# JiehongLin/SAM-6D

Hardware: NVIDIA H100
Metric: poses/sec (higher is better)
Workload: dtype bf16

## Files before the change

### include/sam6d_b200.h

```cpp
#ifndef SAM6D_B200_H
#define SAM6D_B200_H

#ifdef __cplusplus
extern "C" {
#endif


int sam6d_fps(const float* xyz, int b, int n, int m, float* temp, int* idx, void* stream);
int sam6d_fps_single_cta(const float* xyz, int b, int n, int m, float* temp, int* idx, void* stream);

int sam6d_gather_points(const float* points, const int* idx, int b, int c, int n, int m, float* out, void* stream);

int sam6d_gather_rows(const float* src, const int* idx, int b, int n, int m, int c, long long src_bstride, float* out,
                      void* stream);
int sam6d_gather_rows_bf16_f32(const void* src, const int* idx, int b, int n, int m, int c, long long src_bstride, float* out,
                               void* stream);

int sam6d_ball_query(const float* new_xyz, const float* xyz, int b, int n, int m, float radius, int nsample, int* idx,
                     int* cnt, void* stream);
int sam6d_ball_query_pair(const float* new_xyz, const float* xyz, int b, int n, int m, float radius_a, int nsample_a,
                          float radius_b, int nsample_b, int* idx_a, int* idx_b, int* cnt_a, int* cnt_b, void* stream);

int sam6d_group_points(const float* points, const int* idx, int b, int c, int n, int np, int ns, float* out, void* stream);


int sam6d_gemm_f32(const float* A, const float* W, const float* bias, const float* R, float* C, int M, int N, int K,
                   long long lda, long long ldw, long long ldc, long long ldr, int batch, long long sA, long long sW,
                   long long sC, long long sR, float alpha, int relu, void* stream);

int sam6d_gemm_bf16(const void* A, int a_dtype, const void* W, int w_dtype, const float* bias, const float* R, void* C,
                    int c_dtype, int M, int N, int K, long long lda, long long ldw, long long ldc, long long ldr, int batch,
                    long long sA, long long sW, long long sC, long long sR, float alpha, int relu, void* stream);

int sam6d_gemm_tma(const void* A, const void* W, const float* bias, const void* R, void* C, int c_dtype, int M, int N, int K,
                   long long lda, long long ldw, long long ldc, long long ldr, float alpha, int act, void* stream);
int sam6d_gemm_tma_batched(const void* A, const void* W, const float* bias, const void* R, void* C, int c_dtype, int M, int N, int K,
                           long long lda, long long ldw, long long ldc, long long ldr, int batch, long long a_rpb, long long w_rpb,
                           long long c_bs, long long r_bs, float alpha, int act, void* stream);
int sam6d_gemm_tma_vt(const void* A, const void* W, const float* bias, void* C, int M, int N, int K, long long lda, long long ldw,
                      long long ldc, void* Vt, int vt_col0, int vt_S, int vt_N1, void* stream);
int sam6d_gemm_tma_vt2(const void* A, const void* W, const float* bias, void* C, int M, int N, int K, long long lda, long long ldw,
                       long long ldc, void* Vt, int vt_col0, int vt_col1, int vt_S, int vt_N1, void* C2, long long ldc2,
                       void* stream);


int sam6d_layernorm(const float* x, long long x_rpb, long long x_bstride, long long x_ld, float* y, long long y_rpb,
                    long long y_bstride, long long y_ld, const float* gamma, const float* beta, long long rows, int C,
                    float eps, void* stream);
int sam6d_layernorm_bf16(const float* x, long long x_rpb, long long x_bstride, long long x_ld, void* y, long long y_rpb,
                         long long y_bstride, long long y_ld, const float* gamma, const float* beta, long long rows, int C,
                         float eps, void* stream);
int sam6d_layernorm_bf16io(const void* x, long long x_rpb, long long x_bstride, long long x_ld, void* y, long long y_rpb,
                           long long y_bstride, long long y_ld, const float* gamma, const float* beta, long long rows, int C,
                           float eps, void* stream);
int sam6d_l2norm_rows(const float* x, long long x_rpb, long long x_bstride, long long x_ld, float* y, long long y_rpb,
                      long long y_bstride, long long y_ld, long long rows, int C, void* stream);
int sam6d_l2norm_rows_bf16(const float* x, long long x_rpb, long long x_bstride, long long x_ld, void* y, long long y_rpb,
                           long long y_bstride, long long y_ld, long long rows, int C, void* stream);
int sam6d_focus_rows(const float* x, long long x_rpb, long long x_bstride, long long x_ld, float* y, long long y_rpb,
                     long long y_bstride, long long y_ld, const float* softplus_scale, long long rows, int C, void* stream);
int sam6d_rigid_warp(const float* p, const float* R, const float* t, int b, int n, float* out, void* stream);
int sam6d_cloud_radius(const float* po, int b, int n, float* radius, void* stream);
int sam6d_scale_by_radius(const float* src, const float* radius, int b, long long per_batch, float* dst, void* stream);


int sam6d_geo_indices(const float* pts, int b, int S, float sigma_d, float factor_a, float* T, void* stream);
int sam6d_geo_embed_f32(const float* T, long long npairs, const float* div_term, const float* WaT, const float* WdT,
                        const float* bias, float* E, void* stream);

int sam6d_geo_embed_tc(const float* T, long long npairs, const float* div_term, const void* Wa_bf16, const void* Wd_bf16,
                       const float* bias, void* E, int e_is_bf16, void* stream);
int sam6d_geo_embed_dist_tc(const float* T, long long npairs, const float* div_term, const void* Wd_bf16, const float* bias, void* E,
                            void* stream);
int sam6d_geo_embed_lut(const float* T, long long clouds, int S, const void* tabA, int na, float inv_ha, const void* tabD, int nd,
                        float inv_hd, const void* far, const float* div_term, const void* WdT_bf16, const float* bias, void* E,
                        void* stream);


int sam6d_inputs_stage_a(const int* rle_cum, const int* rle_off, int P, int H, int W, const float* depth, double fx, double fy,
                         double cx, double cy, double thr, unsigned char* mask, int* stats, int cap, int* choose1, int* choose2,
                         float* cloud2, void* stream);
int sam6d_inputs_stage_b(const int* stats, const int* keep, int Q, int H, int W, int cap, const int* choose2, const float* cloud2,
                         const int* choose_idx, int ns, int S, const unsigned char* image, const unsigned char* mask, int mask_flag,
                         float* pts, long long* rgb_choose, float* rgb, unsigned char* rgb_u8, void* stream);

int sam6d_crop_resize_normalize(const unsigned char* images, const unsigned char* masks, const int* bbox, int Q, int H, int W, int S,
                                int mask_flag, float* rgb, unsigned char* rgb_u8, void* stream);


int sam6d_crop_resize_pad(const unsigned char* image, const float* masks, const int* boxes, int P, int H, int W, int T, float* rgb,
                          float* pmask, void* stream);
int sam6d_masked_patch_normalize(const float* tokens, long long tok_ld, long long tok_bs, const float* pmask, int P, int G, int patch,
                                 int C, float thresh, float* out_f32, void* out_bf16, unsigned char* valid, void* stream);
int sam6d_appearance_reduce(const float* sim, long long sim_ld, long long sim_bs, int P, int N, const unsigned char* qvalid, float thred,
                            float* appe, float* vis, void* stream);


int sam6d_query_translation(const float* masks, const int* depth, int N, int H, int W, const double* K, double depth_scale,
                            float* translate, void* stream);
int sam6d_project_template_iou(const float* poses, int T, const float* pointcloud, int O, int npc, const long long* best_pose,
                               const long long* pred_obj, const float* translate, const double* K, int N, int H, int W,
                               const long long* boxes, int* image_vu, int* xyxy, float* iou, unsigned char* ok, void* stream);


int sam6d_mask_rle_count(const float* masks, int n, int H, int W, int* col_cnt, int* band_off, int* rle_off, void* stream);
int sam6d_mask_rle_write(const float* masks, int n, int H, int W, const int* col_cnt, const int* band_off, const int* rle_off,
                         int* rle_cum, void* stream);


int sam6d_sam_pe_encode(const float* coords, const float* G, int rows, float* out, void* stream);
int sam6d_sam_mask_embed(const float* masks, const float* params, int B, float* out, void* stream);
int sam6d_sam_self_attn(const float* q, const float* k, const float* v, int B, int T, float* out, void* stream);
int sam6d_sam_tok2img_attn(const float* Q, const void* K, const void* V, long long kv_bs, int B, int T, int L, float* out, void* stream);
int sam6d_sam_img2tok_attn(const void* Q, long long q_bs, const float* Kt, const float* Vt, int B, int T, int L, void* out, void* stream);
int sam6d_sam_ln2d_gelu(const void* x, const float* gamma, const float* beta, long long rows, void* y, void* stream);
int sam6d_sam_mask_dot(const void* up, const float* hyper, int B, int G, float* masks, void* stream);
int sam6d_sam_mask_dot_range(const void* up, const float* hyper, int B, int G, int m0, int nm, float* masks, void* stream);
int sam6d_sam_mask_stats(const float* low, int N, int S, int big, int in_h, int in_w, int H, int W, float thr, float off, int* stats,
                         void* stream);
int sam6d_sam_mask_binarize(const float* low, const int* sel, int K, int S, int big, int in_h, int in_w, int H, int W, float thr,
                            unsigned char* out, void* stream);
int sam6d_sam_mask_upscale(const float* low, int N, int S, int big, int in_h, int in_w, int H, int W, float* out, void* stream);
int sam6d_sam_nms(const float* boxes, int N, float thr, unsigned char* keep, void* stream);


int sam6d_transformer_tail_bf16(const void* hid, long long ld_hid, const void* x, long long ld_x, const void* Wo, const float* bo,
                                const float* g1, const float* b1, const void* We, const float* be, const void* Ws, const float* bs,
                                const float* g2, const float* b2, void* out, long long ld_out, int M, float eps, void* stream);


int sam6d_rpe_scores(const void* E, int e_is_bf16, const float* U, long long u_ld, int B, int S, float* SP, void* stream);
int sam6d_rpe_scores_tc_ld(const void* E, const void* U, int B, int S, float* SP, int sp_ld, void* stream);
int sam6d_mha(const float* Q, long long q_ld, long long q_bs, const float* K, long long k_ld, long long k_bs, const float* V,
              long long v_ld, long long v_bs, const float* bias, int B, int H, int Sq, int Sk, float scale, float* O,
              long long o_ld, long long o_bs, void* stream);
int sam6d_attn_tc(const void* Q, long long q_ld, int q_col0, const void* K, long long k_ld, int k_col0, const void* Vt,
                  long long vt_ld, int B, int H, int Sq, int Sk, int head_dim, int bias_mode, const float* bias,
                  const void* rel_h, const float* rel_w, int Hs, int Ws, const float* bv, float scale, void* out,
                  int out_is_bf16, long long out_ld, void* stream);
int sam6d_attn_tc_bias_ld(const void* Q, long long q_ld, int q_col0, const void* K, long long k_ld, int k_col0, const void* Vt,
                          long long vt_ld, int B, int H, int Sq, int Sk, int head_dim, const float* bias, long long bias_ld,
                          float scale, void* out, int out_is_bf16, long long out_ld, void* stream);
int sam6d_attn_tc_ex(const void* Q, long long q_ld, int q_col0, const void* K, long long k_ld, int k_col0, const void* Vt,
                     long long vt_ld, int B, int H, int Sq, int Sk, int head_dim, float scale, int k_brows, int k_row0, int v_col0,
                     float* lse, void* out, int out_is_bf16, long long out_ld, void* stream);
int sam6d_attn_merge_key(const void* Q, long long q_ld, int q_col0, const void* K, long long k_ld, int k_col0, int k_brows,
                         int key_row, const void* Vt, long long vt_ld, int key_col, const float* lse, int B, int H, int Sq,
                         float scale, void* out, long long out_ld, void* stream);
int sam6d_transpose_tokens_bf16(const void* src, long long ld, int col0, int C, int nB, int L, int N1, void* out, void* stream);
int sam6d_linattn_kv(const float* Kf, long long k_ld, long long k_bs, const float* V, long long v_ld, long long v_bs, int B,
                     int H, int J, float* KV, float* KS, void* stream);
int sam6d_linattn_apply(const float* Qf, long long q_rpb, long long q_bs, long long q_ld, const float* KV, const float* KS,
                        int B, int H, float* X, long long x_bs, long long x_ld, void* stream);
int sam6d_linattn_kv_pack(const float* Kf, long long k_ld, long long k_bs, const float* V, long long v_ld, long long v_bs, int B,
                          int J, void* blob, float* KS, void* stream);
int sam6d_linattn_tc(const void* Q, long long q_ld, long long q_bs, const void* blob, const float* KS,
                     const float* softplus_scale, int B, int rpb, void* X, long long x_ld, long long x_bs, void* stream);

int sam6d_coarse_assign(const float* A, int B, int S, float* W, float* w1, void* stream);
int sam6d_coarse_sample(const float* W, int B, int L, const float* rand, int nr, int* idx, void* stream);
int sam6d_coarse_hypotheses(const int* idx, const float* pts1, const float* pts2, int B, int n, int n1, float* Rt,
                            float* resid, void* stream);
int sam6d_topk_smallest(const float* v, int B, int n, int k, int* out, void* stream);
int sam6d_coarse_select(const float* Rt, const int* top, int B, int n1, int n2, const float* pts1, const float* w1, int n,
                        const float* model, int nm, float* scores, float* R, float* t, void* stream);


int sam6d_pe_mlp_max(const float* pts, const int* idx, const int* cnt, int B, int N, int ns, const float* W1,
                     const float* B1, const float* W2, const float* B2, const float* W3, const float* B3, float* out,
                     int out_ld, int out_off, void* stream);
int sam6d_pe_mlp_max_tc(const float* pts, const int* idx, int B, int N, int ns, const float* W1, const float* B1,
                        const void* W2_bf16, const float* B2, const void* W3_bf16, const float* B3, void* out, int out_is_bf16,
                        int out_ld, int out_off, void* stream);
int sam6d_fine_assign(const float* A, int B, int S, int ld, float shift, const float* pts2, float* rsum, float* csum, float* cpart,
                      int* cpi, int* lab1, int* lab2, float* wts, float* pred, void* stream);
int sam6d_fine_pass_tc(const void* Fa, const void* Fb, int B, int S, float alpha, float shift, int mode, const float* row_f,
                       const float* col_f, int ld_f, const float* q4, float* out_inv, int* lab, float* wts, float* pred, void* stream);
int sam6d_fine_masked_points(const int* lab2, const float* pts2, int B, int S, int ld, float* q4, void* stream);
int sam6d_weighted_procrustes(const float* src, const float* ref, const float* wts, int B, int N, float weight_thresh,
                              float eps, float* R, float* t, void* stream);
int sam6d_pose_score(const float* pts1, const int* lab1, int B, int N, const float* R, const float* t, const float* model,
                     int nm, float dis_thres, const float* radius, float* score, float* t_scaled, void* stream);

int sam6d_bilinear_gather(const void* up, int up_is_bf16, const long long* choose, int B, int K, int G, int sub, int C, int H, int W,
                          float* out, void* stream);

int sam6d_attn_relpos(const float* qkv, long long tok_ld, int nW, int Hs, int Ws, int nH, int head_dim, const float* rel_h,
                      const float* rel_w, float scale, void* out, int out_is_bf16, long long out_ld, void* stream);

int sam6d_attn_global_tc(const void* qkv, long long ld, const void* Vt, long long vt_ld, const void* rel_blob, int B, int H, int grid,
                         float scale, void* out, int out_is_bf16, long long out_ld, void* stream);
int sam6d_attn_global_tc_ex(const void* qkv, long long ld, const void* Vt, long long vt_ld, const void* rel_blob, int B, int H, int grid,
                            int head_dim, float scale, void* out, int out_is_bf16, long long out_ld, void* stream);

int sam6d_template_score(const float* Qn, const float* Rn, int P, int O, int T, int C, float* sim_out, float* obj_score,
                         int* best_obj, float* best_score, int* best_tmpl, void* stream);


int sam6d_render_meshes(const float* verts, const int* faces, const int* mesh_info, int O, int n_verts, int n_faces,
                        const unsigned char* vcol, const float* uv, const unsigned char* tex, const long long* tex_off,
                        const float* base_color, const float* poses, int T, float fx, float fy, float cx, float cy, int H, int W,
                        float znear, float ambient, int* vrec, unsigned long long* vis, int* big, int big_cap, int* counters,
                        unsigned char* rgb, unsigned char* mask, void* xyz, int* tri, float* depth, void* stream);


int sam6d_conv2d_tc(const void* x, long long ldx, int B, int Hi, int Wi, int Cin, const void* w, int k, int stride, int Cout,
                    const float* bias, int silu, const void* r, long long ldr, long long r_bs, void* y, int y_is_f32, long long ldy,
                    long long y_bs, int Wy, int sy, int sx, int oy, int ox, void* stream);
int sam6d_yolo_stem(const unsigned char* img, int B, int H, int W, const float* w, const float* bias, void* out, void* stream);
int sam6d_yolo_sppf(void* buf, long long ld, int B, int H, int W, int C, void* stream);
int sam6d_yolo_upsample2x(const void* x, long long ldx, int B, int H, int W, int C, void* y, long long ldy, void* stream);
int sam6d_yolo_decode(const float* head, long long ld, long long bs, int B, int h0, int w0, int h1, int w1, int h2, int w2, float conf_thr,
                      float* cand, int* count, void* stream);
int sam6d_yolo_masks(const float* proto, int mh, int mw, const float* rows, long long row_ld, int N, int ih, int iw, float kx, float ky,
                     float* low, unsigned char* out, void* stream);

const char* sam6d_version(void);

#ifdef __cplusplus
}
#endif
#endif
```

### sam6d_b200/_lib.py

```python
import ctypes
import os
import re

_HERE = os.path.dirname(os.path.abspath(__file__))
HEADER = os.path.join(os.path.dirname(_HERE), "include", "sam6d_b200.h")
LIB_PATH = os.path.join(_HERE, "libsam6d_b200.so")

_CTYPES = {
    "int": ctypes.c_int,
    "long long": ctypes.c_longlong,
    "float": ctypes.c_float,
    "double": ctypes.c_double,
}


def parse_header(path: str = HEADER):
    text = open(path).read()
    text = re.sub(r"/\*.*?\*/", "", text, flags=re.S)
    protos = {}
    for m in re.finditer(r"(const char\*|int)\s+(sam6d_\w+)\s*\(([^)]*)\)\s*;", text):
        ret, name, args = m.group(1), m.group(2), m.group(3)
        argl = []
        for a in [x.strip() for x in args.split(",")]:
            if a in ("void", ""):
                continue
            if "*" in a:
                argl.append((ctypes.c_void_p, a.split("*")[-1].strip()))
            else:
                typ, nm = a.rsplit(" ", 1)
                argl.append((_CTYPES[typ.strip()], nm))
        protos[name] = (ctypes.c_char_p if ret != "int" else ctypes.c_int, argl)
    return protos


class Sam6dError(RuntimeError):
    pass


_lib = None
_protos = None


def lib():
    global _lib, _protos
    if _lib is None:
        if not os.path.exists(LIB_PATH):
            raise Sam6dError(
                f"{LIB_PATH} not found: build it with `python -m sam6d_b200.build` "
                "(or __graft_entry__.build()); sam6d_b200 has no CPU or eager fallback")
        _lib = ctypes.CDLL(LIB_PATH)
        _protos = parse_header()
        for name, (ret, args) in _protos.items():
            fn = getattr(_lib, name)
            fn.restype = ret
            fn.argtypes = [t for t, _ in args]
    return _lib


_launches = 0
_MULTI = {"sam6d_fine_assign": 6, "sam6d_coarse_select": 2, "sam6d_geo_embed_tc": 2, "sam6d_render_meshes": 4, "sam6d_yolo_masks": 2,
          "sam6d_mask_rle_count": 2}
_timed = {}


def launch_count() -> int:
    return _launches


def add_launches(n: int):
    global _launches
    _launches += int(n)


def time_kernel(name: str, enable: bool = True):
    if enable:
        _timed[name] = []
    else:
        _timed.pop(name, None)


def timed_events(name: str):
    return _timed.get(name, [])


def call(name: str, *args):
    global _launches
    fn = getattr(lib(), name)
    rec = _timed.get(name)
    if rec is not None:
        import torch
        e0, e1 = torch.cuda.Event(enable_timing=True), torch.cuda.Event(enable_timing=True)
        e0.record()
        rc = fn(*args)
        e1.record()
        rec.append((e0, e1))
    else:
        rc = fn(*args)
    _launches += _MULTI.get(name, 1)
    if rc != 0:
        if rc == -22:
            raise Sam6dError(f"{name}: invalid argument (see include/sam6d_b200.h)")
        raise Sam6dError(f"{name}: CUDA error {rc}")
    return rc


def version() -> str:
    return lib().sam6d_version().decode()
```

### sam6d_b200/csrc/fine_tc.cu

```cuda
#include <cuda.h>

#include "common.cuh"
#include "tc.cuh"

namespace {

constexpr int BM = 128, BN = 256, BK = 64, KB = 4, STAGES = 4;
constexpr int A_KB = BM * BK * 2, B_KB = BN * BK * 2;
constexpr int CONSUMERS = 256, NUM_THREADS = CONSUMERS + 128;
constexpr int SMEM_BYTES = KB * A_KB + STAGES * B_KB + 1024;
constexpr float LOG2E = 1.4426950408889634f;

struct FArgs {
  int B, S, mode, ld_f;
  float a2, s2;
  const float* row_f;
  const float* col_f;
  const float4* q4;
  float* out_inv;
  int* lab;
  float* wts; float* pred;
};

__device__ __forceinline__ float ex2(float x) {
  float y;
  asm("ex2.approx.ftz.f32 %0, %1;" : "=f"(y) : "f"(x));
  return y;
}

template <int MODE>
__global__ void __launch_bounds__(NUM_THREADS, 1) fine_pass_kernel(const __grid_constant__ CUtensorMap tmA, const __grid_constant__ CUtensorMap tmB, FArgs g) {
  extern __shared__ __align__(1024) uint8_t smem_raw[];
  uint8_t* smem = reinterpret_cast<uint8_t*>((reinterpret_cast<uintptr_t>(smem_raw) + 1023) & ~(uintptr_t)1023);
  uint8_t* a_res = smem;
  uint8_t* ring = smem + KB * A_KB;
  __shared__ __align__(8) uint64_t a_full, a_empty, full_bar[STAGES], empty_bar[STAGES];
  __shared__ float sc[2][BN];
  __shared__ __align__(16) float4 sq[2][BN];

  const int tid = threadIdx.x, warp = tid >> 5, lane = tid & 31;
  const int m_tiles = (g.S + BM - 1) / BM, n_tiles = (g.S + BN - 1) / BN;
  const int items = g.B * m_tiles;

  if (tid == 0) {
    tc::mbar_init(&a_full, 1); tc::mbar_init(&a_empty, CONSUMERS / 32);
    for (int s = 0; s < STAGES; ++s) { tc::mbar_init(&full_bar[s], 1); tc::mbar_init(&empty_bar[s], CONSUMERS / 32); }
    tc::mbar_fence_init();
    tc::tma_prefetch_desc(&tmA);
    tc::tma_prefetch_desc(&tmB);
  }
  __syncthreads();

  if (warp >= CONSUMERS / 32) {
    tc::producer_regs();
    if (tid == CONSUMERS) {
      long long gk = 0;
      int it = 0;
      for (int item = blockIdx.x; item < items; item += gridDim.x, ++it) {
        const int b = item / m_tiles, mt = item - b * m_tiles;
        tc::mbar_wait(&a_empty, (uint32_t)((it & 1) ^ 1));
        tc::mbar_arrive_expect_tx(&a_full, KB * A_KB);
        for (int kb = 0; kb < KB; ++kb) tc::tma_load_2d(&tmA, &a_full, a_res + kb * A_KB, kb * BK, b * g.S + mt * BM);
        for (int nt = 0; nt < n_tiles; ++nt)
          for (int kb = 0; kb < KB; ++kb, ++gk) {
            const int s = (int)(gk % STAGES);
            tc::mbar_wait(&empty_bar[s], (uint32_t)(((gk / STAGES) & 1) ^ 1));
            tc::mbar_arrive_expect_tx(&full_bar[s], B_KB);
            tc::tma_load_2d(&tmB, &full_bar[s], ring + s * B_KB, kb * BK, b * g.S + nt * BN);
          }
      }
    }
    return;
  }
  tc::consumer_regs();
  const int wg = warp >> 2, w = warp & 3;
  const uint32_t a_addr = tc::smem_u32(a_res) + wg * (64 * 128);
  long long gk = 0, tcount = 0;
  int it = 0;
  for (int item = blockIdx.x; item < items; item += gridDim.x, ++it) {
    const int b = item / m_tiles, mt = item - b * m_tiles;
    float rf[2] = {0.f, 0.f};
#pragma unroll
    for (int hr = 0; hr < 2; ++hr) {
      const int i = mt * BM + wg * 64 + tc::frag_row(2 * hr, w, lane);
      if (MODE != 0 && i < g.S) rf[hr] = g.row_f[(size_t)b * g.ld_f + i];
    }
    const float* cf = (MODE != 0) ? g.col_f + (size_t)b * g.ld_f : nullptr;
    const float4* q4 = (MODE == 2) ? g.q4 + (size_t)b * g.ld_f : nullptr;
    float sum[2] = {0.f, 0.f}, bv[2] = {-INFINITY, -INFINITY}, ws[2] = {0.f, 0.f}, px[2] = {0.f, 0.f}, py[2] = {0.f, 0.f}, pz[2] = {0.f, 0.f};
    int bi[2] = {0x7fffffff, 0x7fffffff};
    tc::mbar_wait(&a_full, (uint32_t)(it & 1));
    for (int nt = 0; nt < n_tiles; ++nt, ++tcount) {
      const int buf = (int)(tcount & 1);
      if (MODE != 0) {
        const int j = nt * BN + tid;
        sc[buf][tid] = (j < g.S) ? cf[j] : 0.f;
        if (MODE == 2) sq[buf][tid] = (j < g.S) ? q4[j] : make_float4(0.f, 0.f, 0.f, 0.f);
        tc::named_bar(1, CONSUMERS);
      }
      float acc[BN / 2];
      int prev = -1;
      for (int kb = 0; kb < KB; ++kb, ++gk) {
        const int s = (int)(gk % STAGES);
        tc::mbar_wait(&full_bar[s], (uint32_t)((gk / STAGES) & 1));
        const uint32_t b_addr = tc::smem_u32(ring + s * B_KB);
        tc::wg_fence();
#pragma unroll
        for (int k = 0; k < BK / 16; ++k)
          tc::wgmma_bf16<BN>(acc, tc::wg_desc(a_addr + kb * A_KB + k * 32), tc::wg_desc(b_addr + k * 32), (kb | k) ? 1u : 0u);
        tc::wg_commit();
        if (prev >= 0) {
          tc::wg_wait<1>();
          if (lane == 0) tc::mbar_arrive(&empty_bar[prev]);
        }
        prev = s;
      }
      tc::wg_wait<0>();
      if (lane == 0) tc::mbar_arrive(&empty_bar[prev]);
      if (nt == n_tiles - 1 && lane == 0) tc::mbar_arrive(&a_empty);
#pragma unroll
      for (int e = 0; e < BN / 2; ++e) {
        const int hr = (e >> 1) & 1, cl = tc::frag_col(e, lane), j = nt * BN + cl;
        const float ev = (j < g.S) ? ex2(fmaf(acc[e], g.a2, -g.s2)) : 0.f;
        if (MODE == 0) {
          sum[hr] += ev;
        } else {
          const float p = (ev * rf[hr]) * (ev * sc[buf][cl]);
          if (p > bv[hr]) { bv[hr] = p; bi[hr] = j; }
          if (MODE == 2) {
            const float4 q = sq[buf][cl];
            const float pm = p * q.w;
            ws[hr] += pm; px[hr] = fmaf(pm, q.x, px[hr]); py[hr] = fmaf(pm, q.y, py[hr]); pz[hr] = fmaf(pm, q.z, pz[hr]);
          }
        }
      }
    }
#pragma unroll
    for (int hr = 0; hr < 2; ++hr) {
      const int i = mt * BM + wg * 64 + tc::frag_row(2 * hr, w, lane);
      if (MODE == 0) {
        const float t = tc::quad_sum(sum[hr]);
        if ((lane & 3) == 0 && i < g.S) g.out_inv[(size_t)b * g.ld_f + i] = 1.f / t;
      } else {
#pragma unroll
        for (int o = 1; o <= 2; o <<= 1) {
          const float ov = __shfl_xor_sync(0xffffffffu, bv[hr], o);
          const int oi = __shfl_xor_sync(0xffffffffu, bi[hr], o);
          if (ov > bv[hr] || (ov == bv[hr] && oi < bi[hr])) { bv[hr] = ov; bi[hr] = oi; }
        }
        float ww = 0.f, qx = 0.f, qy = 0.f, qz = 0.f;
        if (MODE == 2) { ww = tc::quad_sum(ws[hr]); qx = tc::quad_sum(px[hr]); qy = tc::quad_sum(py[hr]); qz = tc::quad_sum(pz[hr]); }
        if ((lane & 3) == 0 && i < g.S) {
          int lb = bi[hr];
          if (lb == 0x7fffffff) lb = 0;
          g.lab[(size_t)b * g.S + i] = lb;
          if (MODE == 2 && i >= 1) {
            if (lb == 0) { ww = 0.f; qx = 0.f; qy = 0.f; qz = 0.f; }
            const size_t o = (size_t)b * (g.S - 1) + (i - 1);
            const float d = ww + 1e-6f;
            g.wts[o] = ww;
            g.pred[o * 3 + 0] = qx / d; g.pred[o * 3 + 1] = qy / d; g.pred[o * 3 + 2] = qz / d;
          }
        }
      }
    }
  }
}

typedef CUresult (*EncodeFn)(CUtensorMap*, CUtensorMapDataType, cuuint32_t, void*, const cuuint64_t*, const cuuint64_t*,
                             const cuuint32_t*, const cuuint32_t*, CUtensorMapInterleave, CUtensorMapSwizzle,
                             CUtensorMapL2promotion, CUtensorMapFloatOOBfill);
EncodeFn f_get_encode() {
  static EncodeFn fn = nullptr;
  if (!fn) {
    void* p = nullptr;
    cudaDriverEntryPointQueryResult q;
    if (cudaGetDriverEntryPoint("cuTensorMapEncodeTiled", &p, cudaEnableDefault, &q) != cudaSuccess || q != cudaDriverEntryPointSuccess)
      return nullptr;
    fn = reinterpret_cast<EncodeFn>(p);
  }
  return fn;
}
int f_make_map(CUtensorMap* map, const void* ptr, long long rows, int box_rows) {
  EncodeFn enc = f_get_encode();
  if (!enc) return 999;
  cuuint64_t gdim[2] = {256, (cuuint64_t)rows};
  cuuint64_t gstride[1] = {512};
  cuuint32_t box[2] = {64, (cuuint32_t)box_rows};
  cuuint32_t estr[2] = {1, 1};
  CUresult r = enc(map, CU_TENSOR_MAP_DATA_TYPE_BFLOAT16, 2, const_cast<void*>(ptr), gdim, gstride, box, estr,
                   CU_TENSOR_MAP_INTERLEAVE_NONE, CU_TENSOR_MAP_SWIZZLE_128B, CU_TENSOR_MAP_L2_PROMOTION_L2_256B,
                   CU_TENSOR_MAP_FLOAT_OOB_FILL_NONE);
  return r == CUDA_SUCCESS ? 0 : 1000 + (int)r;
}

__global__ void fine_masked_points_kernel(const int* __restrict__ lab2, const float* __restrict__ pts2, int S, int ld, float4* __restrict__ q4) {
  const int b = blockIdx.y, j = blockIdx.x * blockDim.x + threadIdx.x;
  if (j >= ld) return;
  float4 q = make_float4(0.f, 0.f, 0.f, 0.f);
  if (j >= 1 && j < S && lab2[(size_t)b * S + j] > 0) {
    const float* p = pts2 + ((size_t)b * (S - 1) + (j - 1)) * 3;
    q = make_float4(p[0], p[1], p[2], 1.f);
  }
  q4[(size_t)b * ld + j] = q;
}

}

S6_API int sam6d_fine_pass_tc(const void* Fa, const void* Fb, int B, int S, float alpha, float shift, int mode, const float* row_f,
                              const float* col_f, int ld_f, const float* q4, float* out_inv, int* lab, float* wts, float* pred,
                              void* stream) {
  S6_REQUIRE(Fa && Fb && B >= 0 && S >= 2 && mode >= 0 && mode <= 2 && ld_f >= S);
  S6_REQUIRE(((reinterpret_cast<uintptr_t>(Fa) | reinterpret_cast<uintptr_t>(Fb)) & 15) == 0 && (long long)B * S < 2000000000LL);
  if (mode == 0) S6_REQUIRE(out_inv != nullptr);
  if (mode >= 1) S6_REQUIRE(row_f && col_f && lab);
  if (mode == 2) S6_REQUIRE(q4 && wts && pred && (reinterpret_cast<uintptr_t>(q4) & 15) == 0);
  if (B == 0) return 0;
  CUtensorMap tmA, tmB;
  int rc = f_make_map(&tmA, Fa, (long long)B * S, BM);
  if (rc) return rc;
  rc = f_make_map(&tmB, Fb, (long long)B * S, BN);
  if (rc) return rc;
  int dev = 0, sms = 0;
  S6_CHECK(cudaGetDevice(&dev));
  S6_CHECK(cudaDeviceGetAttribute(&sms, cudaDevAttrMultiProcessorCount, dev));
  const int items = B * s6_cdiv(S, BM);
  const int grid = items < sms ? items : sms;
  FArgs g{B, S, mode, ld_f, alpha * LOG2E, shift * LOG2E, row_f, col_f, reinterpret_cast<const float4*>(q4), out_inv, lab, wts, pred};
  cudaStream_t st = s6_stream(stream);
#define FINE_LAUNCH(M)                                                                                              \
  do {                                                                                                              \
    S6_CHECK(cudaFuncSetAttribute(fine_pass_kernel<M>, cudaFuncAttributeMaxDynamicSharedMemorySize, SMEM_BYTES));   \
    fine_pass_kernel<M><<<grid, NUM_THREADS, SMEM_BYTES, st>>>(tmA, tmB, g);                                        \
  } while (0)
  if (mode == 0) FINE_LAUNCH(0); else if (mode == 1) FINE_LAUNCH(1); else FINE_LAUNCH(2);
#undef FINE_LAUNCH
  S6_LAUNCH_CHECK();
  return 0;
}

S6_API int sam6d_fine_masked_points(const int* lab2, const float* pts2, int B, int S, int ld, float* q4, void* stream) {
  S6_REQUIRE(lab2 && pts2 && q4 && B >= 0 && S >= 2 && ld >= S && (reinterpret_cast<uintptr_t>(q4) & 15) == 0);
  if (B == 0) return 0;
  dim3 grid(s6_cdiv(ld, 256), B);
  fine_masked_points_kernel<<<grid, 256, 0, s6_stream(stream)>>>(lab2, pts2, S, ld, reinterpret_cast<float4*>(q4));
  S6_LAUNCH_CHECK();
  return 0;
}
```

### sam6d_b200/csrc/pe_tc.cu

```cuda
#include "tc.cuh"

namespace {

constexpr int ROWS = 128;
constexpr int SLAB = ROWS * 128;
constexpr int W2_SLAB = 64 * 128;
constexpr int W3_SLAB = 128 * 128;
constexpr int SMEM_BYTES = 2 * SLAB + W3_SLAB + 1024;
constexpr int NUM_THREADS = 128;

__device__ __forceinline__ void worker_bar() { asm volatile("bar.sync 1, 128;" ::: "memory"); }

__device__ __forceinline__ void st_feat(float* p, float v) { *p = v; }
__device__ __forceinline__ void st_feat(__nv_bfloat16* p, float v) { *p = __float2bfloat16(v); }

template <int NS, typename OT>
__global__ void __launch_bounds__(NUM_THREADS, 4) pe_tc_kernel(const float* __restrict__ pts, const int* __restrict__ idx, int N,
                                                               long long total_points,
                                                               const float* __restrict__ W1, const float* __restrict__ B1,
                                                               const __nv_bfloat16* __restrict__ W2, const float* __restrict__ B2,
                                                               const __nv_bfloat16* __restrict__ W3, const float* __restrict__ B3,
                                                               OT* __restrict__ out, int out_ld, int out_off) {
  extern __shared__ __align__(1024) uint8_t smem_raw[];
  uint8_t* smem = reinterpret_cast<uint8_t*>((reinterpret_cast<uintptr_t>(smem_raw) + 1023) & ~(uintptr_t)1023);
  uint8_t* a1 = smem;
  uint8_t* a2 = a1 + SLAB;
  uint8_t* w3s = a2 + SLAB;
  __shared__ __align__(16) float w1s[32 * 8];
  __shared__ __align__(16) float b1s[32], b2s[64], b3s[128];

  const int tid = threadIdx.x, warp = tid >> 5, lane = tid & 31;
  constexpr int PPT = ROWS / NS;
  const long long ntiles = (total_points + PPT - 1) / PPT;

  for (int e = tid; e < 32 * 8; e += NUM_THREADS) { int r = e >> 3, c = e & 7; w1s[e] = (c < 6) ? W1[r * 6 + c] : 0.f; }
  if (tid < 32) b1s[tid] = B1[tid];
  if (tid < 64) b2s[tid] = B2[tid];
  if (tid < 128) b3s[tid] = B3[tid];
  for (int u = tid; u < 64 * 4; u += NUM_THREADS) {
    const int n = u >> 2, c = (u & 3) << 3;
    *reinterpret_cast<uint4*>(a1 + tc::sw128_offset(n, 32 + c)) = *reinterpret_cast<const uint4*>(W2 + n * 32 + c);
  }
  for (int u = tid; u < 128 * 8; u += NUM_THREADS) {
    const int n = u >> 3, c = (u & 7) << 3;
    *reinterpret_cast<uint4*>(w3s + tc::sw128_offset(n, c)) = *reinterpret_cast<const uint4*>(W3 + n * 64 + c);
  }
  tc::fence_proxy_async_smem();
  __syncthreads();

  {
    const int r = tid;
    const uint32_t a1_addr = tc::smem_u32(a1), a2_addr = tc::smem_u32(a2), w2_addr = tc::smem_u32(a1) + 64, w3_addr = tc::smem_u32(w3s);
    auto load_idx = [&](long long tile) -> int {
      const long long gp = tile * PPT + r / NS;
      return (tile < ntiles && gp < total_points) ? __ldg(idx + gp * NS + (r % NS)) : -1;
    };
    auto load_x = [&](long long tile, int j, float (&xx)[6]) {
      const long long gp = tile * PPT + r / NS;
      if (j >= 0) {
        const long long b = gp / N;
        const float* pi = pts + gp * 3;
        const float* pj = pts + (b * N + j) * 3;
        const float jx = __ldg(pj), jy = __ldg(pj + 1), jz = __ldg(pj + 2);
        xx[0] = jx - __ldg(pi); xx[1] = jy - __ldg(pi + 1); xx[2] = jz - __ldg(pi + 2); xx[3] = jx; xx[4] = jy; xx[5] = jz;
      } else {
#pragma unroll
        for (int e = 0; e < 6; ++e) xx[e] = 0.f;
      }
    };
    float xn[6];
    load_x(blockIdx.x, load_idx(blockIdx.x), xn);
    int jn = load_idx((long long)blockIdx.x + gridDim.x);
    for (long long tile = blockIdx.x; tile < ntiles; tile += gridDim.x) {
      {
        float x[6];
#pragma unroll
        for (int e = 0; e < 6; ++e) x[e] = xn[e];
        uint8_t* row_ptr = a1 + r * 128;
#pragma unroll
        for (int c = 0; c < 4; ++c) {
          uint32_t w[4];
#pragma unroll
          for (int q = 0; q < 4; ++q) {
            float h[2];
#pragma unroll
            for (int e = 0; e < 2; ++e) {
              const int o = c * 8 + q * 2 + e;
              const float4 wa = *reinterpret_cast<const float4*>(&w1s[o * 8]);
              const float2 wb = *reinterpret_cast<const float2*>(&w1s[o * 8 + 4]);
              float a = b1s[o];
              a = fmaf(wa.x, x[0], a); a = fmaf(wa.y, x[1], a); a = fmaf(wa.z, x[2], a);
              a = fmaf(wa.w, x[3], a); a = fmaf(wb.x, x[4], a); a = fmaf(wb.y, x[5], a);
              h[e] = fmaxf(a, 0.f);
            }
            w[q] = tc::pack_bf16(h[0], h[1]);
          }
          *reinterpret_cast<uint4*>(row_ptr + ((c ^ (r & 7)) << 4)) = make_uint4(w[0], w[1], w[2], w[3]);
        }
        tc::fence_proxy_async_smem();
        worker_bar();
      }
#pragma unroll
      for (int blk = 0; blk < 2; ++blk) {
        float acc[32];
        tc::wg_fence();
#pragma unroll
        for (int k = 0; k < 2; ++k)
          tc::wgmma_bf16<64>(acc, tc::wg_desc(a1_addr + blk * (64 * 128) + k * 32), tc::wg_desc(w2_addr + k * 32), k ? 1u : 0u);
        tc::wg_commit();
        tc::wg_wait<0>();
#pragma unroll
        for (int i = 0; i < 32; i += 2) {
          const int row = blk * 64 + tc::frag_row(i, warp, lane), col = tc::frag_col(i, lane);
          *reinterpret_cast<uint32_t*>(a2 + tc::sw128_offset(row, col)) =
              tc::pack_bf16(fmaxf(acc[i] + b2s[col], 0.f), fmaxf(acc[i + 1] + b2s[col + 1], 0.f));
        }
      }
      tc::fence_proxy_async_smem();
      worker_bar();
      load_x(tile + gridDim.x, jn, xn);
      jn = load_idx(tile + 2LL * gridDim.x);
#pragma unroll
      for (int blk = 0; blk < 2; ++blk) {
        float acc[64];
        tc::wg_fence();
#pragma unroll
        for (int k = 0; k < 4; ++k)
          tc::wgmma_bf16<128>(acc, tc::wg_desc(w3_addr + blk * (64 * 128) + k * 32), tc::wg_desc(a2_addr + k * 32), k ? 1u : 0u);
        tc::wg_commit();
        tc::wg_wait<0>();
#pragma unroll
        for (int hr = 0; hr < 2; ++hr) {
          const int ch = blk * 64 + tc::frag_row(2 * hr, warp, lane);
          const float bias = b3s[ch];
#pragma unroll
          for (int p = 0; p < PPT; ++p) {
            constexpr int JG = NS / 8;
            float m = -INFINITY;
#pragma unroll
            for (int j = p * JG; j < (p + 1) * JG; ++j) m = fmaxf(m, fmaxf(acc[4 * j + 2 * hr], acc[4 * j + 2 * hr + 1]));
            m = tc::quad_max(m);
            const long long p_out = tile * PPT + p;
            if ((lane & 3) == 0 && p_out < total_points) st_feat(out + p_out * out_ld + out_off + ch, fmaxf(m + bias, 0.f));
          }
        }
      }
    }
  }
}

}

S6_API int sam6d_pe_mlp_max_tc(const float* pts, const int* idx, int B, int N, int ns, const float* W1, const float* B1,
                               const void* W2_bf16, const float* B2, const void* W3_bf16, const float* B3, void* out, int out_is_bf16,
                               int out_ld, int out_off, void* stream) {
  S6_REQUIRE(pts && idx && W1 && B1 && W2_bf16 && B2 && W3_bf16 && B3 && out && B >= 0 && N > 0);
  S6_REQUIRE(ns == 32 || ns == 64);
  if (B == 0) return 0;
  int dev = 0, sms = 0;
  S6_CHECK(cudaGetDevice(&dev));
  S6_CHECK(cudaDeviceGetAttribute(&sms, cudaDevAttrMultiProcessorCount, dev));
  const long long total = (long long)B * N;
  const long long ntiles = (total + (128 / ns) - 1) / (128 / ns);
  cudaStream_t st = s6_stream(stream);
  const __nv_bfloat16* W2 = reinterpret_cast<const __nv_bfloat16*>(W2_bf16);
  const __nv_bfloat16* W3 = reinterpret_cast<const __nv_bfloat16*>(W3_bf16);
#define PE_LAUNCH(NSV, OT)                                                                                                          \
  do {                                                                                                                              \
    S6_CHECK(cudaFuncSetAttribute(pe_tc_kernel<NSV, OT>, cudaFuncAttributeMaxDynamicSharedMemorySize, SMEM_BYTES));                 \
                       \
    S6_CHECK(cudaFuncSetAttribute(pe_tc_kernel<NSV, OT>, cudaFuncAttributePreferredSharedMemoryCarveout, 100));                     \
       \
       \
    const int per_sm = 4;                                                                                                           \
    const int grid = (int)(ntiles < (long long)sms * per_sm ? ntiles : (long long)sms * per_sm);                                    \
    pe_tc_kernel<NSV, OT><<<grid, NUM_THREADS, SMEM_BYTES, st>>>(pts, idx, N, total, W1, B1, W2, B2, W3, B3,                         \
                                                                 reinterpret_cast<OT*>(out), out_ld, out_off);                      \
  } while (0)
  if (ns == 32) { if (out_is_bf16) PE_LAUNCH(32, __nv_bfloat16); else PE_LAUNCH(32, float); }
  else { if (out_is_bf16) PE_LAUNCH(64, __nv_bfloat16); else PE_LAUNCH(64, float); }
#undef PE_LAUNCH
  S6_LAUNCH_CHECK();
  return 0;
}
```

### sam6d_b200/ops.py

```python
import ctypes
from typing import Optional, Tuple

import torch

from . import _lib

Tensor = torch.Tensor


def _check(t: Tensor, dtype, name: str, ndim: Optional[int] = None):
    if not isinstance(t, torch.Tensor):
        raise RuntimeError(f"{name} must be a torch.Tensor")
    if not t.is_cuda:
        raise RuntimeError(f"{name} must be a CUDA tensor (CPU not supported)")
    if t.dtype != dtype:
        raise RuntimeError(f"{name} must be {dtype}, got {t.dtype}")
    if not t.is_contiguous():
        raise RuntimeError(f"{name} must be contiguous")
    if ndim is not None and t.dim() != ndim:
        raise RuntimeError(f"{name} must have {ndim} dims, got {t.dim()}")


def _p(t: Optional[Tensor]):
    return ctypes.c_void_p(0 if t is None else t.data_ptr())


def _s():
    return ctypes.c_void_p(torch.cuda.current_stream().cuda_stream)


def _ll(v):
    return ctypes.c_longlong(int(v))


def _f(v):
    return ctypes.c_float(float(v))


def furthest_point_sampling(xyz: Tensor, m: int) -> Tensor:
    _check(xyz, torch.float32, "points", 3)
    b, n, c = xyz.shape
    if c != 3:
        raise RuntimeError("points must be (B,N,3)")
    idx = torch.zeros(b, m, dtype=torch.int32, device=xyz.device)
    temp = torch.empty(b, n, dtype=torch.float32, device=xyz.device) if n > 4096 else None
    _lib.call("sam6d_fps", _p(xyz), b, n, int(m), _p(temp), _p(idx), _s())
    return idx


def furthest_point_sampling_single_cta(xyz: Tensor, m: int) -> Tensor:
    _check(xyz, torch.float32, "points", 3)
    b, n, _ = xyz.shape
    idx = torch.zeros(b, m, dtype=torch.int32, device=xyz.device)
    temp = torch.empty(b, n, dtype=torch.float32, device=xyz.device)
    _lib.call("sam6d_fps_single_cta", _p(xyz), b, n, int(m), _p(temp), _p(idx), _s())
    return idx


def gather_points(points: Tensor, idx: Tensor) -> Tensor:
    _check(points, torch.float32, "points", 3)
    _check(idx, torch.int32, "idx", 2)
    b, c, n = points.shape
    m = idx.shape[1]
    out = torch.zeros(b, c, m, dtype=torch.float32, device=points.device)
    _lib.call("sam6d_gather_points", _p(points), _p(idx), b, c, n, m, _p(out), _s())
    return out


def gather_rows(src: Tensor, idx: Tensor, n_rows: Optional[int] = None) -> Tensor:
    _check(src, torch.float32, "src", 3)
    _check(idx, torch.int32, "idx", 2)
    b, n, c = src.shape
    m = idx.shape[1]
    out = torch.empty(b, m, c, dtype=torch.float32, device=src.device)
    _lib.call("sam6d_gather_rows", _p(src), _p(idx), b, n, m, c, _ll(n * c), _p(out), _s())
    return out


def ball_query(new_xyz: Tensor, xyz: Tensor, radius: float, nsample: int, return_count: bool = False):
    _check(new_xyz, torch.float32, "new_xyz", 3)
    _check(xyz, torch.float32, "xyz", 3)
    b, m, _ = new_xyz.shape
    n = xyz.shape[1]
    idx = torch.zeros(b, m, nsample, dtype=torch.int32, device=xyz.device)
    cnt = torch.zeros(b, m, dtype=torch.int32, device=xyz.device) if return_count else None
    _lib.call("sam6d_ball_query", _p(new_xyz), _p(xyz), b, n, m, _f(radius), int(nsample), _p(idx), _p(cnt), _s())
    return (idx, cnt) if return_count else idx


def ball_query_pair(new_xyz: Tensor, xyz: Tensor, ra: float, nsa: int, rb: float, nsb: int):
    _check(new_xyz, torch.float32, "new_xyz", 3)
    _check(xyz, torch.float32, "xyz", 3)
    b, m, _ = new_xyz.shape
    n = xyz.shape[1]
    dev = xyz.device
    ia = torch.empty(b, m, nsa, dtype=torch.int32, device=dev)
    ib = torch.empty(b, m, nsb, dtype=torch.int32, device=dev)
    ca = torch.empty(b, m, dtype=torch.int32, device=dev)
    cb = torch.empty(b, m, dtype=torch.int32, device=dev)
    _lib.call("sam6d_ball_query_pair", _p(new_xyz), _p(xyz), b, n, m, _f(ra), int(nsa), _f(rb), int(nsb), _p(ia), _p(ib), _p(ca),
              _p(cb), _s())
    return ia, ca, ib, cb


def group_points(points: Tensor, idx: Tensor) -> Tensor:
    _check(points, torch.float32, "points", 3)
    _check(idx, torch.int32, "idx", 3)
    b, c, n = points.shape
    _, npnt, ns = idx.shape
    out = torch.zeros(b, c, npnt, ns, dtype=torch.float32, device=points.device)
    _lib.call("sam6d_group_points", _p(points), _p(idx), b, c, n, npnt, ns, _p(out), _s())
    return out


def gemm(A: Tensor, W: Tensor, bias: Optional[Tensor] = None, residual: Optional[Tensor] = None,
         out: Optional[Tensor] = None, relu=False, alpha: float = 1.0) -> Tensor:
    _check(A, torch.float32, "A", 2)
    _check(W, torch.float32, "W", 2)
    M, K = A.shape
    N = W.shape[0]
    if W.shape[1] != K:
        raise RuntimeError("gemm: inner dimensions differ")
    if out is None:
        out = torch.empty(M, N, dtype=torch.float32, device=A.device)
    _lib.call("sam6d_gemm_f32", _p(A), _p(W), _p(bias), _p(residual), _p(out), M, N, K, _ll(K), _ll(K), _ll(N), _ll(N),
              1, _ll(0), _ll(0), _ll(0), _ll(0), _f(alpha), int(relu), _s())
    return out


def gemm_raw(A_ptr, W_ptr, bias, R_ptr, C_ptr, M, N, K, lda, ldw, ldc, ldr, batch=1, sA=0, sW=0, sC=0, sR=0,
             alpha=1.0, relu=False):
    _lib.call("sam6d_gemm_f32", ctypes.c_void_p(A_ptr), ctypes.c_void_p(W_ptr), _p(bias), ctypes.c_void_p(R_ptr or 0),
              ctypes.c_void_p(C_ptr), int(M), int(N), int(K), _ll(lda), _ll(ldw), _ll(ldc), _ll(ldr), int(batch), _ll(sA),
              _ll(sW), _ll(sC), _ll(sR), _f(alpha), int(relu), _s())


_DT = {torch.float32: 0, torch.bfloat16: 1}


def gemm_tc_raw(A_ptr, a_dt, W_ptr, w_dt, bias, R_ptr, C_ptr, c_dt, M, N, K, lda, ldw, ldc, ldr, batch=1, sA=0, sW=0, sC=0, sR=0,
                alpha=1.0, relu=False):
    _lib.call("sam6d_gemm_bf16", ctypes.c_void_p(A_ptr), int(a_dt), ctypes.c_void_p(W_ptr), int(w_dt), _p(bias),
              ctypes.c_void_p(R_ptr or 0), ctypes.c_void_p(C_ptr), int(c_dt), int(M), int(N), int(K), _ll(lda), _ll(ldw), _ll(ldc),
              _ll(ldr), int(batch), _ll(sA), _ll(sW), _ll(sC), _ll(sR), _f(alpha), int(relu), _s())


def gemm_tc(A: Tensor, W: Tensor, bias: Optional[Tensor] = None, residual: Optional[Tensor] = None, out: Optional[Tensor] = None,
            relu: bool = False, alpha: float = 1.0, out_dtype=torch.float32) -> Tensor:
    for t, n in ((A, "A"), (W, "W")):
        if t.dtype not in _DT:
            raise RuntimeError(f"{n} must be float32 or bfloat16")
        _check(t, t.dtype, n, 2)
    M, K = A.shape
    N = W.shape[0]
    if W.shape[1] != K:
        raise RuntimeError("gemm: inner dimensions differ")
    if out is None:
        out = torch.empty(M, N, dtype=out_dtype, device=A.device)
    gemm_tc_raw(A.data_ptr(), _DT[A.dtype], W.data_ptr(), _DT[W.dtype], bias, residual.data_ptr() if residual is not None else 0,
                out.data_ptr(), _DT[out.dtype], M, N, K, K, K, N, N, alpha=alpha, relu=relu)
    return out


def gemm_tma(A: Tensor, W: Tensor, bias: Optional[Tensor] = None, residual: Optional[Tensor] = None, out: Optional[Tensor] = None,
             act: int = 0, alpha: float = 1.0, out_dtype=torch.float32) -> Tensor:
    _check(A, torch.bfloat16, "A", 2)
    _check(W, torch.bfloat16, "W", 2)
    M, K = A.shape
    N = W.shape[0]
    if W.shape[1] != K:
        raise RuntimeError("gemm: inner dimensions differ")
    Nout = N // 2 if act == ACT_SWIGLU else N
    if out is None:
        out = torch.empty(M, Nout, dtype=torch.bfloat16 if act == ACT_SWIGLU else out_dtype, device=A.device)
    if residual is not None:
        _check(residual, out.dtype, "residual", 2)
    _lib.call("sam6d_gemm_tma", _p(A), _p(W), _p(bias), _p(residual), _p(out), _DT[out.dtype], M, N, K, _ll(K), _ll(K), _ll(Nout), _ll(N),
              _f(alpha), int(act), _s())
    return out


ACT_SWIGLU = 3


def pack_swiglu_rows(t: Tensor, block: int = 128) -> Tensor:
    H = t.shape[0] // 2
    if t.shape[0] != 2 * H or H % block:
        raise ValueError(f"SwiGLU w12 needs 2H rows with H % {block} == 0, got {t.shape[0]}")
    rest = t.shape[1:]
    return t.reshape(2, H // block, block, *rest).transpose(0, 1).reshape(2 * H, *rest).contiguous()


_VT_CACHE = {}


def _vt_buffer(rows: int, n1: int, device, slot: int) -> Tensor:
    key = (rows, n1, str(device), slot, torch.cuda.current_stream(device).cuda_stream)
    buf = _VT_CACHE.get(key)
    if buf is None:
        if len(_VT_CACHE) > 64:
            _VT_CACHE.clear()
        buf = torch.zeros(rows, n1, dtype=torch.bfloat16, device=device)
        _VT_CACHE[key] = buf
    return buf


def gemm_tma_vt(A: Tensor, W: Tensor, bias: Tensor, vt_col0: int, S: int, slot: int = 0) -> Tuple[Tensor, Tensor]:
    _check(A, torch.bfloat16, "A", 2)
    _check(W, torch.bfloat16, "W", 2)
    M, K = A.shape
    N = W.shape[0]
    if W.shape[1] != K or M % S or not (0 < vt_col0 < N):
        raise RuntimeError("gemm_tma_vt: shape mismatch")
    n1 = (S + 15) // 16 * 16
    out = torch.empty(M, vt_col0, dtype=torch.bfloat16, device=A.device)
    vt = _vt_buffer((M // S) * (N - vt_col0), n1, A.device, slot)
    _lib.call("sam6d_gemm_tma_vt", _p(A), _p(W), _p(bias), _p(out), M, N, K, _ll(K), _ll(K), _ll(vt_col0), _p(vt), int(vt_col0), int(S),
              int(n1), _s())
    return out, vt


def gemm_tma_vt2(A: Tensor, W: Tensor, bias: Tensor, vt_col0: int, vt_col1: int, S: int, slot: int = 0) -> Tuple[Tensor, Tensor, Tensor]:
    _check(A, torch.bfloat16, "A", 2)
    _check(W, torch.bfloat16, "W", 2)
    M, K = A.shape
    N = W.shape[0]
    if W.shape[1] != K or M % S or not (0 < vt_col0 < vt_col1 < N):
        raise RuntimeError("gemm_tma_vt2: shape mismatch")
    n1 = (S + 15) // 16 * 16
    out = torch.empty(M, vt_col0, dtype=torch.bfloat16, device=A.device)
    out2 = torch.empty(M, N - vt_col1, dtype=torch.bfloat16, device=A.device)
    vt = _vt_buffer((M // S) * (vt_col1 - vt_col0), n1, A.device, slot)
    _lib.call("sam6d_gemm_tma_vt2", _p(A), _p(W), _p(bias), _p(out), M, N, K, _ll(K), _ll(K), _ll(vt_col0), _p(vt), int(vt_col0),
              int(vt_col1), int(S), int(n1), _p(out2), _ll(N - vt_col1), _s())
    return out, vt, out2


def layernorm_raw(x_ptr, x_view, y_ptr, y_view, gamma: Tensor, beta: Tensor, rows: int, C: int, eps: float = 1e-5):
    _lib.call("sam6d_layernorm", ctypes.c_void_p(x_ptr), _ll(x_view[0]), _ll(x_view[1]), _ll(x_view[2]),
              ctypes.c_void_p(y_ptr), _ll(y_view[0]), _ll(y_view[1]), _ll(y_view[2]), _p(gamma), _p(beta), _ll(rows), int(C),
              _f(eps), _s())


def layernorm(x: Tensor, gamma: Tensor, beta: Tensor, eps: float = 1e-5, out: Optional[Tensor] = None) -> Tensor:
    _check(x, torch.float32, "x")
    C = x.shape[-1]
    rows = x.numel() // C
    if out is None:
        out = torch.empty_like(x)
    layernorm_raw(x.data_ptr(), (rows, 0, C), out.data_ptr(), (rows, 0, C), gamma, beta, rows, C, eps)
    return out


def layernorm_bf16(x: Tensor, gamma: Tensor, beta: Tensor, eps: float = 1e-5) -> Tensor:
    _check(x, torch.float32, "x")
    C = x.shape[-1]
    rows = x.numel() // C
    out = torch.empty(x.shape, dtype=torch.bfloat16, device=x.device)
    _lib.call("sam6d_layernorm_bf16", _p(x), _ll(rows), _ll(0), _ll(C), _p(out), _ll(rows), _ll(0), _ll(C), _p(gamma), _p(beta),
              _ll(rows), int(C), _f(eps), _s())
    return out


def layernorm_bf16io(x: Tensor, gamma: Tensor, beta: Tensor, eps: float = 1e-5, out: Optional[Tensor] = None) -> Tensor:
    _check(x, torch.bfloat16, "x")
    C = x.shape[-1]
    rows = x.numel() // C
    if out is None:
        out = torch.empty_like(x)
    _lib.call("sam6d_layernorm_bf16io", _p(x), _ll(max(rows, 1)), _ll(0), _ll(C), _p(out), _ll(max(rows, 1)), _ll(0), _ll(C),
              _p(gamma), _p(beta), _ll(rows), int(C), _f(eps), _s())
    return out


def transformer_tail_bf16(hid: Tensor, x: Tensor, wo: Tensor, bo: Tensor, g1: Tensor, b1: Tensor, we: Tensor, be: Tensor, ws: Tensor,
                          bs: Tensor, g2: Tensor, b2: Tensor, out: Optional[Tensor] = None, eps: float = 1e-5) -> Tensor:
    _check(hid, torch.bfloat16, "hid", 2)
    _check(x, torch.bfloat16, "x", 2)
    M = hid.shape[0]
    if hid.shape[1] != 256 or x.shape != hid.shape or wo.shape != (256, 256) or we.shape != (512, 256) or ws.shape != (256, 512):
        raise RuntimeError("transformer_tail_bf16: d_model 256, hidden 512")
    for w in (wo, we, ws):
        _check(w, torch.bfloat16, "weight", 2)
    if out is None:
        out = torch.empty_like(hid)
    _check(out, torch.bfloat16, "out", 2)
    _lib.call("sam6d_transformer_tail_bf16", _p(hid), _ll(256), _p(x), _ll(256), _p(wo), _p(bo), _p(g1), _p(b1), _p(we), _p(be), _p(ws),
              _p(bs), _p(g2), _p(b2), _p(out), _ll(256), int(M), _f(eps), _s())
    return out


def gather_rows_bf16_f32(src: Tensor, idx: Tensor) -> Tensor:
    _check(src, torch.bfloat16, "src", 3)
    _check(idx, torch.int32, "idx", 2)
    b, n, c = src.shape
    m = idx.shape[1]
    out = torch.empty(b, m, c, dtype=torch.float32, device=src.device)
    _lib.call("sam6d_gather_rows_bf16_f32", _p(src), _p(idx), b, n, m, c, _ll(n * c), _p(out), _s())
    return out


def gather_rows_bf16(src: Tensor, idx: Tensor) -> Tensor:
    _check(src, torch.bfloat16, "src", 3)
    _check(idx, torch.int32, "idx", 2)
    b, n, c = src.shape
    m = idx.shape[1]
    out = torch.empty(b, m, c, dtype=torch.bfloat16, device=src.device)
    _lib.call("sam6d_gather_rows", _p(src), _p(idx), b, n, m, c // 2, _ll(n * c // 2), _p(out), _s())
    return out


def l2norm_rows(x: Tensor) -> Tensor:
    _check(x, torch.float32, "x")
    C = x.shape[-1]
    rows = x.numel() // C
    out = torch.empty_like(x)
    _lib.call("sam6d_l2norm_rows", _p(x), _ll(rows), _ll(0), _ll(C), _p(out), _ll(rows), _ll(0), _ll(C), _ll(rows), C, _s())
    return out


def l2norm_rows_bf16(x: Tensor) -> Tensor:
    _check(x, torch.float32, "x")
    C = x.shape[-1]
    rows = x.numel() // C
    out = torch.empty(x.shape, dtype=torch.bfloat16, device=x.device)
    _lib.call("sam6d_l2norm_rows_bf16", _p(x), _ll(max(rows, 1)), _ll(0), _ll(C), _p(out), _ll(max(rows, 1)), _ll(0), _ll(C), _ll(rows), C,
              _s())
    return out


def gemm_tma_batched(A: Tensor, W: Tensor, out: Tensor, M: int, N: int, ldc: int, c_bs: int, alpha: float = 1.0,
                     bias: Optional[Tensor] = None, residual: Optional[Tensor] = None, ldr: int = 0, r_bs: int = 0) -> Tensor:
    _check(A, torch.bfloat16, "A", 3)
    _check(W, torch.bfloat16, "W")
    batch, a_rows, K = A.shape
    shared = W.dim() == 2
    if W.shape[-1] != K or a_rows < M or (not shared and (W.shape[0] != batch or W.shape[1] < N)) or (shared and W.shape[0] != N):
        raise RuntimeError("gemm_tma_batched: shape mismatch")
    if residual is not None and residual.dtype != out.dtype:
        raise RuntimeError("gemm_tma_batched: the residual must have the output's element type")
    _lib.call("sam6d_gemm_tma_batched", _p(A), _p(W), _p(bias), _p(residual), _p(out), _DT[out.dtype], int(M), int(N), int(K), _ll(K),
              _ll(K), _ll(ldc), _ll(ldr), int(batch), _ll(a_rows), _ll(0 if shared else W.shape[1]), _ll(c_bs), _ll(r_bs), _f(alpha), 0,
              _s())
    return out


def focus_rows_raw(x_ptr, x_view, y_ptr, y_view, sp_scale: Tensor, rows: int, C: int):
    _lib.call("sam6d_focus_rows", ctypes.c_void_p(x_ptr), _ll(x_view[0]), _ll(x_view[1]), _ll(x_view[2]),
              ctypes.c_void_p(y_ptr), _ll(y_view[0]), _ll(y_view[1]), _ll(y_view[2]), _p(sp_scale), _ll(rows), int(C), _s())


def rigid_warp(p: Tensor, R: Tensor, t: Tensor) -> Tensor:
    _check(p, torch.float32, "p", 3)
    _check(R, torch.float32, "R", 3)
    _check(t, torch.float32, "t", 2)
    out = torch.empty_like(p)
    _lib.call("sam6d_rigid_warp", _p(p), _p(R), _p(t), p.shape[0], p.shape[1], _p(out), _s())
    return out


def cloud_radius(po: Tensor) -> Tensor:
    _check(po, torch.float32, "dense_po", 3)
    r = torch.empty(po.shape[0], dtype=torch.float32, device=po.device)
    _lib.call("sam6d_cloud_radius", _p(po), po.shape[0], po.shape[1], _p(r), _s())
    return r


def scale_by_radius(x: Tensor, radius: Tensor) -> Tensor:
    _check(x, torch.float32, "x")
    _check(radius, torch.float32, "radius", 1)
    out = torch.empty_like(x)
    b = x.shape[0]
    _lib.call("sam6d_scale_by_radius", _p(x), _p(radius), b, _ll(x.numel() // max(b, 1)), _p(out), _s())
    return out


def geo_indices(pts: Tensor, sigma_d: float, factor_a: float) -> Tensor:
    _check(pts, torch.float32, "points", 3)
    b, s, _ = pts.shape
    T = torch.empty(b, s, s, 4, dtype=torch.float32, device=pts.device)
    _lib.call("sam6d_geo_indices", _p(pts), b, s, _f(sigma_d), _f(factor_a), _p(T), _s())
    return T


def geo_embed_f32(T: Tensor, div_term: Tensor, WaT: Tensor, WdT: Tensor, bias: Tensor) -> Tensor:
    _check(T, torch.float32, "T", 4)
    b, s, _, _ = T.shape
    E = torch.empty(b, s, s, 256, dtype=torch.float32, device=T.device)
    _lib.call("sam6d_geo_embed_f32", _p(T), _ll(b * s * s), _p(div_term), _p(WaT), _p(WdT), _p(bias), _p(E), _s())
    return E


def geo_embed_tc(T: Tensor, div_term: Tensor, Wa_bf16: Tensor, Wd_bf16: Tensor, bias: Tensor, out_dtype=torch.bfloat16) -> Tensor:
    _check(T, torch.float32, "T", 4)
    _check(Wa_bf16, torch.bfloat16, "Wa", 2)
    _check(Wd_bf16, torch.bfloat16, "Wd", 2)
    b, s, _, _ = T.shape
    E = torch.empty(b, s, s, 256, dtype=out_dtype, device=T.device)
    _lib.call("sam6d_geo_embed_tc", _p(T), _ll(b * s * s), _p(div_term), _p(Wa_bf16), _p(Wd_bf16), _p(bias), _p(E),
              int(out_dtype == torch.bfloat16), _s())
    return E


def geo_embed_dist_tc(T: Tensor, div_term: Tensor, Wd_bf16: Tensor, bias: Tensor) -> Tensor:
    if T.dtype != torch.float32 or not T.is_cuda or not T.is_contiguous() or T.shape[-1] != 4:
        raise RuntimeError("T must be a contiguous CUDA float32 tensor (..., 4)")
    _check(Wd_bf16, torch.bfloat16, "Wd", 2)
    n = T.numel() // 4
    E = torch.empty(*T.shape[:-1], 256, dtype=torch.bfloat16, device=T.device)
    _lib.call("sam6d_geo_embed_dist_tc", _p(T), _ll(n), _p(div_term), _p(Wd_bf16), _p(bias), _p(E), _s())
    return E


def geo_embed_lut(T: Tensor, tabA: Tensor, inv_ha: float, tabD: Tensor, inv_hd: float, far: Tensor, div_term: Tensor, WdT_bf16: Tensor,
                  bias: Tensor) -> Tensor:
    _check(T, torch.float32, "T", 4)
    _check(tabA, torch.bfloat16, "tabA", 2)
    _check(tabD, torch.bfloat16, "tabD", 2)
    _check(far, torch.bfloat16, "far", 4)
    _check(WdT_bf16, torch.bfloat16, "WdT", 2)
    b, s, _, _ = T.shape
    if far.shape != (b, 2, s, 256) or tabA.shape[1] != 256 or tabD.shape[1] != 256 or T.shape[3] != 4:
        raise RuntimeError("geo_embed_lut: shape mismatch")
    E = torch.empty(b, s, s, 256, dtype=torch.bfloat16, device=T.device)
    _lib.call("sam6d_geo_embed_lut", _p(T), _ll(b), s, _p(tabA), tabA.shape[0], _f(inv_ha), _p(tabD), tabD.shape[0], _f(inv_hd), _p(far),
              _p(div_term), _p(WdT_bf16), _p(bias), _p(E), _s())
    return E


def rpe_scores(E: Tensor, U: Tensor, u_ptr: Optional[int] = None, u_ld: int = 1024) -> Tensor:
    if E.dtype not in (torch.float32, torch.bfloat16):
        raise RuntimeError("E must be float32 or bfloat16")
    _check(E, E.dtype, "E", 4)
    if u_ptr is None:
        _check(U, torch.float32, "U", 4)
        u_ptr = U.data_ptr()
    B, S = E.shape[0], E.shape[1]
    SP = torch.empty(B, 4, S, S, dtype=torch.float32, device=E.device)
    _lib.call("sam6d_rpe_scores", _p(E), int(E.dtype == torch.bfloat16), ctypes.c_void_p(u_ptr), _ll(u_ld), B, S, _p(SP), _s())
    return SP


def rpe_scores_tc(E: Tensor, U: Tensor, ld: Optional[int] = None) -> Tensor:
    _check(E, torch.bfloat16, "E", 4)
    _check(U, torch.bfloat16, "U", 2)
    B, S = E.shape[0], E.shape[1]
    if U.shape != (B * S, 1024) or E.shape[3] != 256 or E.shape[2] != S:
        raise RuntimeError("rpe_scores_tc: E (B,S,S,256), U (B*S,1024)")
    ld = S if ld is None else ld
    SP = torch.empty(B, 4, S, ld, dtype=torch.float32, device=E.device)
    _lib.call("sam6d_rpe_scores_tc_ld", _p(E), _p(U), B, S, _p(SP), int(ld), _s())
    return SP


def rpe_scores_tc_padded(E: Tensor, U: Tensor) -> Tensor:
    return rpe_scores_tc(E, U, ld=(E.shape[1] + 15) // 16 * 16)


def attn_tc_padded_bias(Q: Tensor, q_col0: int, K: Tensor, k_col0: int, Vt: Tensor, B: int, H: int, Sq: int, Sk: int, D: int,
                        scale: float, bias: Tensor, out_dtype=torch.bfloat16) -> Tensor:
    _check(Q, torch.bfloat16, "Q", 2)
    _check(K, torch.bfloat16, "K", 2)
    _check(Vt, torch.bfloat16, "Vt", 2)
    _check(bias, torch.float32, "bias", 4)
    if bias.shape[:3] != (B, H, Sq) or bias.shape[3] < Sk or bias.shape[3] % 4:
        raise RuntimeError("attn_tc_padded_bias: bias (B,H,Sq,ld), ld >= Sk, ld % 4 == 0")
    out = torch.empty(B * Sq, H * D, dtype=out_dtype, device=Q.device)
    _lib.call("sam6d_attn_tc_bias_ld", _p(Q), _ll(Q.shape[1]), int(q_col0), _p(K), _ll(K.shape[1]), int(k_col0), _p(Vt), _ll(Vt.shape[1]),
              int(B), int(H), int(Sq), int(Sk), int(D), _p(bias), _ll(bias.shape[3]), _f(scale), _p(out),
              int(out_dtype == torch.bfloat16), _ll(H * D), _s())
    return out


def mha_raw(q_ptr, q_ld, q_bs, k_ptr, k_ld, k_bs, v_ptr, v_ld, v_bs, bias: Optional[Tensor], B, H, Sq, Sk, scale,
            o_ptr, o_ld, o_bs):
    _lib.call("sam6d_mha", ctypes.c_void_p(q_ptr), _ll(q_ld), _ll(q_bs), ctypes.c_void_p(k_ptr), _ll(k_ld), _ll(k_bs),
              ctypes.c_void_p(v_ptr), _ll(v_ld), _ll(v_bs), _p(bias), int(B), int(H), int(Sq), int(Sk), _f(scale),
              ctypes.c_void_p(o_ptr), _ll(o_ld), _ll(o_bs), _s())


def pack_rel_pos(rel_h: Tensor, rel_w: Tensor, slab_rows: int = 32) -> Tensor:
    D = rel_h.shape[1]
    DS = (D + 63) // 64
    if rel_h.shape[0] > slab_rows or rel_w.shape[0] > slab_rows:
        raise RuntimeError("pack_rel_pos: table has more rows than the slab")
    blob = torch.zeros(2 * DS * slab_rows * 64, dtype=torch.bfloat16, device=rel_h.device)
    j = torch.arange(slab_rows, device=rel_h.device).view(slab_rows, 1)
    c = torch.arange(D, device=rel_h.device).view(1, D)
    off = j * 64 + ((((c % 64) // 8) ^ (j % 8)) * 8) + (c % 8)
    for t, tab in enumerate((rel_h, rel_w)):
        n = tab.shape[0]
        idx = ((t * DS + c // 64) * slab_rows * 64 + off)[:n]
        blob[idx.reshape(-1)] = tab.to(torch.bfloat16).reshape(-1)
    return blob


def attn_global_tc(qkv: Tensor, vt: Tensor, rel_blob: Tensor, B: int, H: int, grid: int, scale: float, out_dtype=torch.bfloat16,
                   D: int = 80) -> Tensor:
    _check(qkv, torch.bfloat16, "qkv", 2)
    _check(vt, torch.bfloat16, "vt", 2)
    _check(rel_blob, torch.bfloat16, "rel_blob", 1)
    L = grid * grid
    out = torch.empty(B * L, H * D, dtype=out_dtype, device=qkv.device)
    _lib.call("sam6d_attn_global_tc_ex", _p(qkv), _ll(qkv.shape[1]), _p(vt), _ll(vt.shape[1]), _p(rel_blob), int(B), int(H), int(grid),
              int(D), _f(scale), _p(out), int(out_dtype == torch.bfloat16), _ll(H * D), _s())
    return out


def attn_tc(Q: Tensor, q_col0: int, K: Tensor, k_col0: int, Vt: Tensor, B: int, H: int, Sq: int, Sk: int, D: int, scale: float,
            bias: Optional[Tensor] = None, rel: Optional[tuple] = None, bv: Optional[Tensor] = None,
            out_dtype=torch.float32) -> Tensor:
    _check(Q, torch.bfloat16, "Q", 2)
    _check(K, torch.bfloat16, "K", 2)
    _check(Vt, torch.bfloat16, "Vt", 2)
    mode, rh, rw, Hs, Ws = 0, None, None, 0, 0
    if bias is not None:
        _check(bias, torch.float32, "bias", 4)
        mode = 1
    elif rel is not None:
        rh, Hs, Ws = rel
        mode = 2
    out = torch.empty(B * Sq, H * D, dtype=out_dtype, device=Q.device)
    _lib.call("sam6d_attn_tc", _p(Q), _ll(Q.shape[1]), int(q_col0), _p(K), _ll(K.shape[1]), int(k_col0), _p(Vt), _ll(Vt.shape[1]),
              int(B), int(H), int(Sq), int(Sk), int(D), mode, _p(bias), _p(rh), _p(rw), int(Hs), int(Ws), _p(bv), _f(scale), _p(out),
              int(out_dtype == torch.bfloat16), _ll(H * D), _s())
    return out


def attn_tc_ex(Q: Tensor, q_col0: int, K: Tensor, k_col0: int, Vt: Tensor, B: int, H: int, Sq: int, Sk: int, D: int, scale: float,
               k_brows: int, k_row0: int = 0, v_col0: int = 0, want_lse: bool = False, out_dtype=torch.bfloat16):
    _check(Q, torch.bfloat16, "Q", 2)
    _check(K, torch.bfloat16, "K", 2)
    _check(Vt, torch.bfloat16, "Vt", 2)
    out = torch.empty(B * Sq, H * D, dtype=out_dtype, device=Q.device)
    lse = torch.empty(B, H, Sq, dtype=torch.float32, device=Q.device) if want_lse else None
    _lib.call("sam6d_attn_tc_ex", _p(Q), _ll(Q.shape[1]), int(q_col0), _p(K), _ll(K.shape[1]), int(k_col0), _p(Vt), _ll(Vt.shape[1]),
              int(B), int(H), int(Sq), int(Sk), int(D), _f(scale), int(k_brows), int(k_row0), int(v_col0), _p(lse), _p(out),
              int(out_dtype == torch.bfloat16), _ll(H * D), _s())
    return out, lse


def attn_merge_key(Q: Tensor, q_col0: int, K: Tensor, k_col0: int, k_brows: int, key_row: int, Vt: Tensor, key_col: int, lse: Tensor,
                   B: int, H: int, Sq: int, scale: float, out: Tensor) -> Tensor:
    _check(out, torch.bfloat16, "out", 2)
    _check(lse, torch.float32, "lse", 3)
    _lib.call("sam6d_attn_merge_key", _p(Q), _ll(Q.shape[1]), int(q_col0), _p(K), _ll(K.shape[1]), int(k_col0), int(k_brows), int(key_row),
              _p(Vt), _ll(Vt.shape[1]), int(key_col), _p(lse), int(B), int(H), int(Sq), _f(scale), _p(out), _ll(out.shape[1]), _s())
    return out


def transpose_tokens(src: Tensor, col0: int, C: int, nB: int, L: int) -> Tensor:
    _check(src, torch.bfloat16, "src", 2)
    N1 = (L + 15) // 16 * 16
    out = torch.empty(nB * C, N1, dtype=torch.bfloat16, device=src.device)
    _lib.call("sam6d_transpose_tokens_bf16", _p(src), _ll(src.shape[1]), int(col0), int(C), int(nB), int(L), int(N1), _p(out), _s())
    return out


def linattn_kv_raw(k_ptr, k_ld, k_bs, v_ptr, v_ld, v_bs, B, H, J, KV: Tensor, KS: Tensor):
    _lib.call("sam6d_linattn_kv", ctypes.c_void_p(k_ptr), _ll(k_ld), _ll(k_bs), ctypes.c_void_p(v_ptr), _ll(v_ld), _ll(v_bs),
              int(B), int(H), int(J), _p(KV), _p(KS), _s())


def linattn_apply_raw(q_ptr, q_rpb, q_bs, q_ld, KV: Tensor, KS: Tensor, B, H, x_ptr, x_bs, x_ld):
    _lib.call("sam6d_linattn_apply", ctypes.c_void_p(q_ptr), _ll(q_rpb), _ll(q_bs), _ll(q_ld), _p(KV), _p(KS), int(B), int(H),
              ctypes.c_void_p(x_ptr), _ll(x_bs), _ll(x_ld), _s())


def linattn_kv_pack_raw(k_ptr, k_ld, k_bs, v_ptr, v_ld, v_bs, B, J, device):
    blob = torch.empty(B, 4 * 64 * 64, dtype=torch.bfloat16, device=device)
    KS = torch.empty(B, 4, 64, dtype=torch.float32, device=device)
    _lib.call("sam6d_linattn_kv_pack", ctypes.c_void_p(k_ptr), _ll(k_ld), _ll(k_bs), ctypes.c_void_p(v_ptr), _ll(v_ld), _ll(v_bs),
              int(B), int(J), _p(blob), _p(KS), _s())
    return blob, KS


def linattn_tc_raw(q_ptr, q_ld, q_bs, blob: Tensor, KS: Tensor, sp_scale: Tensor, B, rpb, x_ptr, x_ld, x_bs):
    _lib.call("sam6d_linattn_tc", ctypes.c_void_p(q_ptr), _ll(q_ld), _ll(q_bs), _p(blob), _p(KS), _p(sp_scale), int(B), int(rpb),
              ctypes.c_void_p(x_ptr), _ll(x_ld), _ll(x_bs), _s())


def coarse_assign(A: Tensor) -> Tuple[Tensor, Tensor]:
    _check(A, torch.float32, "atten", 3)
    B, S, _ = A.shape
    n = S - 1
    W = torch.empty(B, n * n, dtype=torch.float32, device=A.device)
    w1 = torch.empty(B, n, dtype=torch.float32, device=A.device)
    _lib.call("sam6d_coarse_assign", _p(A), B, S, _p(W), _p(w1), _s())
    return W, w1


def coarse_sample(W: Tensor, rand: Tensor) -> Tensor:
    _check(W, torch.float32, "W", 2)
    _check(rand, torch.float32, "rand", 2)
    B, L = W.shape
    nr = rand.shape[1]
    idx = torch.empty(B, nr, dtype=torch.int32, device=W.device)
    _lib.call("sam6d_coarse_sample", _p(W), B, L, _p(rand), nr, _p(idx), _s())
    return idx


def coarse_hypotheses(idx: Tensor, pts1: Tensor, pts2: Tensor) -> Tuple[Tensor, Tensor]:
    _check(idx, torch.int32, "idx", 2)
    _check(pts1, torch.float32, "pts1", 3)
    _check(pts2, torch.float32, "pts2", 3)
    B, n, _ = pts1.shape
    n1 = idx.shape[1] // 3
    Rt = torch.empty(B, n1, 12, dtype=torch.float32, device=idx.device)
    resid = torch.empty(B, n1, dtype=torch.float32, device=idx.device)
    _lib.call("sam6d_coarse_hypotheses", _p(idx), _p(pts1), _p(pts2), B, n, n1, _p(Rt), _p(resid), _s())
    return Rt, resid


def topk_smallest(v: Tensor, k: int) -> Tensor:
    _check(v, torch.float32, "v", 2)
    B, n = v.shape
    out = torch.empty(B, k, dtype=torch.int32, device=v.device)
    _lib.call("sam6d_topk_smallest", _p(v), B, n, int(k), _p(out), _s())
    return out


def coarse_select(Rt: Tensor, top: Tensor, pts1: Tensor, w1: Tensor, model: Tensor):
    _check(Rt, torch.float32, "Rt", 3)
    _check(top, torch.int32, "top", 2)
    _check(model, torch.float32, "model", 3)
    B, n1, _ = Rt.shape
    n2 = top.shape[1]
    n = pts1.shape[1]
    scores = torch.empty(B, n2, dtype=torch.float32, device=Rt.device)
    R = torch.empty(B, 3, 3, dtype=torch.float32, device=Rt.device)
    t = torch.empty(B, 3, dtype=torch.float32, device=Rt.device)
    _lib.call("sam6d_coarse_select", _p(Rt), _p(top), B, n1, n2, _p(pts1), _p(w1), n, _p(model), model.shape[1], _p(scores),
              _p(R), _p(t), _s())
    return R, t, scores


def pe_mlp_max(pts: Tensor, idx: Tensor, cnt: Tensor, weights, out: Tensor, out_off: int):
    _check(pts, torch.float32, "pts", 3)
    _check(idx, torch.int32, "idx", 3)
    _check(cnt, torch.int32, "cnt", 2)
    B, N, _ = pts.shape
    ns = idx.shape[2]
    W1, B1, W2, B2, W3, B3 = weights
    _lib.call("sam6d_pe_mlp_max", _p(pts), _p(idx), _p(cnt), B, N, ns, _p(W1), _p(B1), _p(W2), _p(B2), _p(W3), _p(B3),
              _p(out), out.shape[-1], int(out_off), _s())


def pe_mlp_max_tc(pts: Tensor, idx: Tensor, weights, out: Tensor, out_off: int):
    _check(pts, torch.float32, "pts", 3)
    _check(idx, torch.int32, "idx", 3)
    B, N, _ = pts.shape
    ns = idx.shape[2]
    W1, B1, W2, B2, W3, B3 = weights
    _check(W2, torch.bfloat16, "W2", 2)
    _check(W3, torch.bfloat16, "W3", 2)
    if out.dtype not in (torch.float32, torch.bfloat16):
        raise RuntimeError("pe_mlp_max_tc: out must be float32 or bfloat16")
    _lib.call("sam6d_pe_mlp_max_tc", _p(pts), _p(idx), B, N, ns, _p(W1), _p(B1), _p(W2), _p(B2), _p(W3), _p(B3), _p(out),
              int(out.dtype == torch.bfloat16), out.shape[-1], int(out_off), _s())


def fine_assign(A: Tensor, pts2: Tensor, shift: float):
    if A.dim() != 3 or A.dtype != torch.float32 or not A.is_cuda:
        raise RuntimeError("atten must be a CUDA fp32 (B,S,S) tensor")
    _check(pts2, torch.float32, "pts2", 3)
    B, S, _ = A.shape
    if A.stride(2) != 1 or A.stride(0) != S * A.stride(1) or A.stride(1) % 4 or A.data_ptr() % 16:
        ld = (S + 3) // 4 * 4
        store = torch.empty(B, S, ld, dtype=torch.float32, device=A.device)
        store[:, :, :S] = A
        A = store[:, :, :S]
    ld = A.stride(1)
    dev = A.device
    tiles = (S + 31) // 32
    if tiles < 4:
        raise RuntimeError("fine_assign: S >= 97 required")
    rsum = torch.empty(B, ld, dtype=torch.float32, device=dev)
    csum = torch.empty(B, ld, dtype=torch.float32, device=dev)
    cpart = torch.empty(B, tiles, ld, dtype=torch.float32, device=dev)
    cpi = torch.empty(B, tiles, ld, dtype=torch.int32, device=dev)
    lab1 = torch.zeros(B, S, dtype=torch.int32, device=dev)
    lab2 = torch.zeros(B, S, dtype=torch.int32, device=dev)
    wts = torch.empty(B, S - 1, dtype=torch.float32, device=dev)
    pred = torch.empty(B, S - 1, 3, dtype=torch.float32, device=dev)
    _lib.call("sam6d_fine_assign", _p(A), B, S, int(ld), _f(shift), _p(pts2), _p(rsum), _p(csum), _p(cpart), _p(cpi), _p(lab1),
              _p(lab2), _p(wts), _p(pred), _s())
    return lab1, lab2, wts, pred


def fine_assign_tc(f1n: Tensor, f2n: Tensor, pts2: Tensor, alpha: float):
    _check(f1n, torch.bfloat16, "f1n", 3)
    _check(f2n, torch.bfloat16, "f2n", 3)
    _check(pts2, torch.float32, "pts2", 3)
    B, S, C = f1n.shape
    if C != 256 or f2n.shape != f1n.shape or pts2.shape[1] != S - 1:
        raise RuntimeError("fine_assign_tc: (B,S,256) tokens and (B,S-1,3) points expected")
    dev = f1n.device
    ld = (S + 3) // 4 * 4
    rinv = torch.empty(B, ld, dtype=torch.float32, device=dev)
    cinv = torch.empty(B, ld, dtype=torch.float32, device=dev)
    q4 = torch.empty(B, ld, 4, dtype=torch.float32, device=dev)
    lab1 = torch.zeros(B, S, dtype=torch.int32, device=dev)
    lab2 = torch.zeros(B, S, dtype=torch.int32, device=dev)
    wts = torch.empty(B, S - 1, dtype=torch.float32, device=dev)
    pred = torch.empty(B, S - 1, 3, dtype=torch.float32, device=dev)
    a, sh = _f(alpha), _f(alpha)
    _lib.call("sam6d_fine_pass_tc", _p(f1n), _p(f2n), B, S, a, sh, 0, None, None, ld, None, _p(rinv), None, None, None, _s())
    _lib.call("sam6d_fine_pass_tc", _p(f2n), _p(f1n), B, S, a, sh, 0, None, None, ld, None, _p(cinv), None, None, None, _s())
    _lib.call("sam6d_fine_pass_tc", _p(f2n), _p(f1n), B, S, a, sh, 1, _p(cinv), _p(rinv), ld, None, None, _p(lab2), None, None, _s())
    _lib.call("sam6d_fine_masked_points", _p(lab2), _p(pts2), B, S, ld, _p(q4), _s())
    _lib.call("sam6d_fine_pass_tc", _p(f1n), _p(f2n), B, S, a, sh, 2, _p(rinv), _p(cinv), ld, _p(q4), None, _p(lab1), _p(wts), _p(pred),
              _s())
    return lab1, lab2, wts, pred


def weighted_procrustes(src: Tensor, ref: Tensor, wts: Tensor, weight_thresh: float = 0.0, eps: float = 1e-5):
    _check(src, torch.float32, "src", 3)
    _check(ref, torch.float32, "ref", 3)
    _check(wts, torch.float32, "weights", 2)
    B, N, _ = src.shape
    R = torch.empty(B, 3, 3, dtype=torch.float32, device=src.device)
    t = torch.empty(B, 3, dtype=torch.float32, device=src.device)
    _lib.call("sam6d_weighted_procrustes", _p(src), _p(ref), _p(wts), B, N, _f(weight_thresh), _f(eps), _p(R), _p(t), _s())
    return R, t


def pose_score(pts1: Tensor, lab1: Tensor, R: Tensor, t: Tensor, model: Tensor, radius: Tensor, dis_thres: float = 0.15):
    _check(pts1, torch.float32, "pts1", 3)
    _check(lab1, torch.int32, "lab1", 2)
    B, N, _ = pts1.shape
    score = torch.empty(B, dtype=torch.float32, device=pts1.device)
    ts = torch.empty(B, 3, dtype=torch.float32, device=pts1.device)
    _lib.call("sam6d_pose_score", _p(pts1), _p(lab1), B, N, _p(R), _p(t), _p(model), model.shape[1], _f(dis_thres),
              _p(radius), _p(score), _p(ts), _s())
    return score, ts


def attn_relpos(qkv: Tensor, nW: int, Hs: int, Ws: int, nH: int, rel_h: Tensor, rel_w: Tensor, scale: float,
                out_dtype=torch.float32) -> Tensor:
    _check(qkv, torch.float32, "qkv", 2)
    _check(rel_h, torch.float32, "rel_pos_h", 2)
    _check(rel_w, torch.float32, "rel_pos_w", 2)
    T, C3 = qkv.shape
    C = C3 // 3
    if T != nW * Hs * Ws or rel_h.shape[0] != 2 * Hs - 1 or rel_w.shape[0] != 2 * Ws - 1:
        raise RuntimeError("attn_relpos: shape mismatch")
    out = torch.empty(T, C, dtype=out_dtype, device=qkv.device)
    _lib.call("sam6d_attn_relpos", _p(qkv), _ll(C3), int(nW), int(Hs), int(Ws), int(nH), C // nH, _p(rel_h), _p(rel_w), _f(scale),
              _p(out), int(out_dtype == torch.bfloat16), _ll(C), _s())
    return out


def bilinear_gather(up: Tensor, choose: Tensor, G: int, sub: int, C: int, H: int, W: int) -> Tensor:
    if up.dtype not in (torch.float32, torch.bfloat16):
        raise RuntimeError("bilinear_gather: up must be float32 or bfloat16")
    _check(up, up.dtype, "up", 3)
    _check(choose, torch.int64, "choose", 2)
    B, K = choose.shape
    if up.shape != (B, G * G, sub * sub * C):
        raise RuntimeError("bilinear_gather: shape mismatch")
    out = torch.empty(B, K, C, dtype=torch.float32, device=up.device)
    _lib.call("sam6d_bilinear_gather", _p(up), int(up.dtype == torch.bfloat16), _p(choose), int(B), int(K), int(G), int(sub), int(C),
              int(H), int(W), _p(out), _s())
    return out


def template_score(Qn: Tensor, Rn: Tensor, want_sim: bool = True):
    _check(Qn, torch.float32, "query", 2)
    _check(Rn, torch.float32, "reference", 3)
    P, C = Qn.shape
    O, T, _ = Rn.shape
    dev = Qn.device
    sim = torch.empty(P, O, T, dtype=torch.float32, device=dev) if want_sim else None
    obj = torch.empty(P, O, dtype=torch.float32, device=dev)
    bo = torch.zeros(P, dtype=torch.int32, device=dev)
    bs = torch.zeros(P, dtype=torch.float32, device=dev)
    bt = torch.zeros(P, dtype=torch.int32, device=dev)
    _lib.call("sam6d_template_score", _p(Qn), _p(Rn), P, O, T, C, _p(sim), _p(obj), _p(bo), _p(bs), _p(bt), _s())
    return sim, obj, bo, bs, bt


def mask_rle(masks: Tensor) -> Tuple[Tensor, Tensor]:
    _check(masks, torch.float32, "masks", 3)
    n, H, W = masks.shape
    dev = masks.device
    col_cnt = torch.empty(n, W, dtype=torch.int32, device=dev)
    band_off = torch.empty(n, (W + 31) // 32, dtype=torch.int32, device=dev)
    rle_off = torch.empty(n + 1, dtype=torch.int32, device=dev)
    _lib.call("sam6d_mask_rle_count", _p(masks), n, H, W, _p(col_cnt), _p(band_off), _p(rle_off), _s())
    rle_cum = torch.empty(int(rle_off[n]), dtype=torch.int32, device=dev)
    _lib.call("sam6d_mask_rle_write", _p(masks), n, H, W, _p(col_cnt), _p(band_off), _p(rle_off), _p(rle_cum), _s())
    return rle_cum, rle_off
```

### sam6d_b200/pem.py

```python
import math
from types import SimpleNamespace
from typing import Dict, Optional

import torch
import torch.nn as nn

from . import ops

NUM_HEADS = 4

PRECISIONS = ("fp32", "bf16")
RPE_TC = True
PADDED_BIAS = True
GEO_LUT_INV_H = 8.0
GEO_LUT_D_MAX = 32.0


class _W:
    __slots__ = ("f32", "bf16")

    def __init__(self, w: torch.Tensor):
        self.f32 = w.detach().to(torch.float32).contiguous()
        self.bf16 = self.f32.to(torch.bfloat16).contiguous()


def _gemm(prec, A, W: "_W", bias=None, residual=None, relu=False):
    if prec == "bf16":
        if A.dtype == torch.bfloat16 and residual is None and A.is_contiguous() and A.shape[1] % 64 == 0:
            return ops.gemm_tma(A, W.bf16, bias, act=1 if relu else 0)
        return ops.gemm_tc(A, W.bf16, bias, residual=residual, relu=relu)
    return ops.gemm(A, W.f32, bias, residual=residual, relu=relu)


def _gemm_raw(prec, A_ptr, W: "_W", bias, R_ptr, C_ptr, M, N, K, lda, ldc, ldr=0, batch=1, sA=0, sC=0, sR=0):
    if prec == "bf16":
        ops.gemm_tc_raw(A_ptr, 0, W.bf16.data_ptr(), 1, bias, R_ptr, C_ptr, 0, M, N, K, lda, K, ldc, ldr, batch=batch, sA=sA, sW=0,
                        sC=sC, sR=sR)
    else:
        ops.gemm_raw(A_ptr, W.f32.data_ptr(), bias, R_ptr, C_ptr, M, N, K, lda, K, ldc, ldr, batch=batch, sA=sA, sW=0, sC=sC, sR=sR)


def _cfg(cfg, **defaults):
    if isinstance(cfg, dict):
        cfg = SimpleNamespace(**cfg)
    for k, v in defaults.items():
        if not hasattr(cfg, k):
            setattr(cfg, k, v)
    return cfg


class _MHAParams(nn.Module):
    def __init__(self, d_model, rpe: bool):
        super().__init__()
        self.proj_q = nn.Linear(d_model, d_model)
        self.proj_k = nn.Linear(d_model, d_model)
        self.proj_v = nn.Linear(d_model, d_model)
        if rpe:
            self.proj_p = nn.Linear(d_model, d_model)


class _AttentionLayerParams(nn.Module):
    def __init__(self, d_model, rpe: bool):
        super().__init__()
        self.attention = _MHAParams(d_model, rpe)
        self.linear = nn.Linear(d_model, d_model)
        self.norm = nn.LayerNorm(d_model)


class _AttentionOutputParams(nn.Module):
    def __init__(self, d_model):
        super().__init__()
        self.expand = nn.Linear(d_model, d_model * 2)
        self.squeeze = nn.Linear(d_model * 2, d_model)
        self.norm = nn.LayerNorm(d_model)


class _TransformerLayerParams(nn.Module):
    def __init__(self, d_model, rpe: bool):
        super().__init__()
        self.attention = _AttentionLayerParams(d_model, rpe)
        self.output = _AttentionOutputParams(d_model)


class _Packed:

    def __init__(self):
        self.key = None
        self.w = {}


def _param_key(module: nn.Module):
    return tuple((p.data_ptr(), p._version) for p in module.parameters()) + tuple(
        (b.data_ptr(), b._version) for b in module.buffers())


def _f32(t: torch.Tensor) -> torch.Tensor:
    return t.detach().to(torch.float32).contiguous()


def _stack2(a: torch.Tensor, b: torch.Tensor) -> Optional[torch.Tensor]:
    if (a.shape == b.shape and a.dtype == b.dtype and a.is_contiguous() and b.is_contiguous() and a.device == b.device
            and a.untyped_storage().data_ptr() == b.untyped_storage().data_ptr()
            and b.storage_offset() == a.storage_offset() + a.numel()):
        return torch.as_strided(a, (2 * a.shape[0],) + tuple(a.shape[1:]), a.stride(), a.storage_offset())
    return None


def _attn_tail(prec, x2d: torch.Tensor, hid: torch.Tensor, lw) -> torch.Tensor:
    y = _gemm(prec, hid, lw["wo"], lw["bo"], residual=x2d)
    y = ops.layernorm(y, lw["g1"], lw["b1"])
    h = _gemm(prec, y, lw["we"], lw["be"], relu=True)
    z = _gemm(prec, h, lw["ws"], lw["bs"], residual=y)
    return ops.layernorm(z, lw["g2"], lw["b2"])


def _pack_tail(layer: nn.Module) -> Dict[str, torch.Tensor]:
    a, o = layer.attention, layer.output
    return dict(wo=_W(a.linear.weight), bo=_f32(a.linear.bias), g1=_f32(a.norm.weight), b1=_f32(a.norm.bias),
                we=_W(o.expand.weight), be=_f32(o.expand.bias), ws=_W(o.squeeze.weight), bs=_f32(o.squeeze.bias),
                g2=_f32(o.norm.weight), b2=_f32(o.norm.bias))


def _tail_bf16(x2d: torch.Tensor, hid: torch.Tensor, lw, out: Optional[torch.Tensor] = None) -> torch.Tensor:
    return ops.transformer_tail_bf16(hid, x2d, lw["wo"].bf16, lw["bo"], lw["g1"], lw["b1"], lw["we"].bf16, lw["be"],
                                     lw["ws"].bf16, lw["bs"], lw["g2"], lw["b2"], out=out)


class GeometricTransformer(nn.Module):

    def __init__(self, blocks, d_model, num_heads, dropout=None, activation_fn='ReLU', return_attention_scores=False,
                 parallel=False):
        super().__init__()
        if list(blocks) != ['self', 'cross'] or parallel or return_attention_scores or dropout:
            raise ValueError("sam6d_b200.GeometricTransformer supports the configuration SAM-6D uses: "
                             "blocks=['self','cross'], parallel=False, dropout=None, no attention-score output")
        if activation_fn != 'ReLU' or num_heads != NUM_HEADS or d_model != 256:
            raise ValueError("sam6d_b200 kernels are built for d_model=256, num_heads=4, ReLU")
        self.blocks = list(blocks)
        self.d_model, self.num_heads = d_model, num_heads
        self.layers = nn.ModuleList([_TransformerLayerParams(d_model, rpe=True), _TransformerLayerParams(d_model, rpe=False)])
        self._packed = _Packed()
        self.precision = "fp32"

    def _weights(self):
        key = _param_key(self)
        if self._packed.key != key:
            C, H = self.d_model, self.num_heads
            d = C // H
            sa = self.layers[0].attention.attention
            wq, bq = _f32(sa.proj_q.weight), _f32(sa.proj_q.bias)
            wp = _f32(sa.proj_p.weight)
            mu = [wp[h * d:(h + 1) * d, :].t().double() @ wq[h * d:(h + 1) * d, :].double() for h in range(H)]
            cu = [wp[h * d:(h + 1) * d, :].t().double() @ bq[h * d:(h + 1) * d].double() for h in range(H)]
            w_self = torch.cat([wq, _f32(sa.proj_k.weight), _f32(sa.proj_v.weight)] + [m.float() for m in mu], dim=0)
            b_self = torch.cat([bq, _f32(sa.proj_k.bias), _f32(sa.proj_v.bias)] + [c.float() for c in cu], dim=0)
            ca = self.layers[1].attention.attention
            self._packed.w = dict(
                w_self=_W(w_self), b_self=b_self.contiguous(), tail_self=_pack_tail(self.layers[0]),
                w_qkv=_W(w_self[:3 * C]), b_qkv=b_self[:3 * C].contiguous(), w_u=_W(w_self[3 * C:]), b_u=b_self[3 * C:].contiguous(),
                wq_c=_W(ca.proj_q.weight), bq_c=_f32(ca.proj_q.bias),
                wkv_c=_W(torch.cat([_f32(ca.proj_k.weight), _f32(ca.proj_v.weight)], dim=0)),
                bkv_c=torch.cat([_f32(ca.proj_k.bias), _f32(ca.proj_v.bias)], dim=0).contiguous(),
                wkqv_c=_W(torch.cat([_f32(ca.proj_k.weight), _f32(ca.proj_q.weight), _f32(ca.proj_v.weight)], dim=0)),
                bkqv_c=torch.cat([_f32(ca.proj_k.bias), _f32(ca.proj_q.bias), _f32(ca.proj_v.bias)], dim=0).contiguous(),
                tail_cross=_pack_tail(self.layers[1]))
            self._packed.key = key
        return self._packed.w

    def _self_layer(self, x: torch.Tensor, emb: torch.Tensor, w) -> torch.Tensor:
        B, S, C = x.shape
        x2d = x.reshape(B * S, C)
        if self.precision == "bf16" and S <= 256:
            d = C // NUM_HEADS
            qkv = ops.gemm_tc(x2d, w["w_qkv"].bf16, w["b_qkv"], out_dtype=torch.bfloat16)
            u = ops.gemm_tc(x2d, w["w_u"].bf16, w["b_u"])
            sp = ops.rpe_scores(emb, None, u_ptr=u.data_ptr(), u_ld=NUM_HEADS * C)
            vt = ops.transpose_tokens(qkv, 2 * C, C, B, S)
            hid = ops.attn_tc(qkv, 0, qkv, C, vt, B, NUM_HEADS, S, S, d, 1.0 / math.sqrt(d), bias=sp)
            return _attn_tail(self.precision, x2d, hid, w["tail_self"]).view(B, S, C)
        ld = 3 * C + NUM_HEADS * C
        qkvu = _gemm(self.precision, x2d, w["w_self"], w["b_self"])
        base, f = qkvu.data_ptr(), 4
        sp = ops.rpe_scores(emb, None, u_ptr=base + 3 * C * f, u_ld=ld)
        hid = torch.empty(B * S, C, dtype=torch.float32, device=x.device)
        ops.mha_raw(base, ld, S * ld, base + C * f, ld, S * ld, base + 2 * C * f, ld, S * ld, sp, B, NUM_HEADS, S, S,
                    1.0 / math.sqrt(C // NUM_HEADS), hid.data_ptr(), C, S * C)
        return _attn_tail(self.precision, x2d, hid, w["tail_self"]).view(B, S, C)

    def _cross_layer(self, x: torch.Tensor, mem: torch.Tensor, w) -> torch.Tensor:
        B, S, C = x.shape
        Sm = mem.shape[1]
        x2d = x.reshape(B * S, C)
        if self.precision == "bf16" and Sm <= 256:
            d = C // NUM_HEADS
            q = ops.gemm_tc(x2d, w["wq_c"].bf16, w["bq_c"], out_dtype=torch.bfloat16)
            kv = ops.gemm_tc(mem.reshape(B * Sm, C), w["wkv_c"].bf16, w["bkv_c"], out_dtype=torch.bfloat16)
            vt = ops.transpose_tokens(kv, C, C, B, Sm)
            hid = ops.attn_tc(q, 0, kv, 0, vt, B, NUM_HEADS, S, Sm, d, 1.0 / math.sqrt(d))
            return _attn_tail(self.precision, x2d, hid, w["tail_cross"]).view(B, S, C)
        q = _gemm(self.precision, x2d, w["wq_c"], w["bq_c"])
        kv = _gemm(self.precision, mem.reshape(B * Sm, C), w["wkv_c"], w["bkv_c"])
        hid = torch.empty(B * S, C, dtype=torch.float32, device=x.device)
        ops.mha_raw(q.data_ptr(), C, S * C, kv.data_ptr(), 2 * C, Sm * 2 * C, kv.data_ptr() + C * 4, 2 * C, Sm * 2 * C, None,
                    B, NUM_HEADS, S, Sm, 1.0 / math.sqrt(C // NUM_HEADS), hid.data_ptr(), C, S * C)
        return _attn_tail(self.precision, x2d, hid, w["tail_cross"]).view(B, S, C)

    def _self_bf16(self, x, emb, w):
        B, S, C = x.shape
        d = C // NUM_HEADS
        x2d = x.view(B * S, C)
        if S <= 200 and emb.dtype == torch.bfloat16:
            qk, vt, u = ops.gemm_tma_vt2(x2d, w["w_self"].bf16, w["b_self"], 2 * C, 3 * C, S)
            sp = ops.rpe_scores_tc_padded(emb, u)
            hid = ops.attn_tc_padded_bias(qk, 0, qk, C, vt, B, NUM_HEADS, S, S, d, 1.0 / math.sqrt(d), sp)
            return _tail_bf16(x2d, hid, w["tail_self"]).view(B, S, C)
        qk, vt = ops.gemm_tma_vt(x2d, w["w_qkv"].bf16, w["b_qkv"], 2 * C, S)
        u = ops.gemm_tma(x2d, w["w_u"].bf16, w["b_u"])
        sp = ops.rpe_scores(emb, None, u_ptr=u.data_ptr(), u_ld=NUM_HEADS * C)
        hid = ops.attn_tc(qk, 0, qk, C, vt, B, NUM_HEADS, S, S, d, 1.0 / math.sqrt(d), bias=sp, out_dtype=torch.bfloat16)
        return _tail_bf16(x2d, hid, w["tail_self"]).view(B, S, C)

    def _forward_bf16(self, f, emb, w):
        B, S, C = f.shape[0] // 2, f.shape[1], f.shape[2]
        d = C // NUM_HEADS
        scale = 1.0 / math.sqrt(d)
        f = self._self_bf16(f, emb, w)
        out = torch.empty_like(f)
        x0, x1 = f[:B].view(B * S, C), f[B:].view(B * S, C)
        kq, vt_all = ops.gemm_tma_vt(f.view(2 * B * S, C), w["wkqv_c"].bf16, w["bkqv_c"], 2 * C, S, slot=1)
        kq1, vt1 = kq[B * S:], vt_all[B * C:]
        hid = ops.attn_tc(kq, C, kq1, 0, vt1, B, NUM_HEADS, S, S, d, scale, out_dtype=torch.bfloat16)
        _tail_bf16(x0, hid, w["tail_cross"], out=out[:B].view(B * S, C))
        k0, vt0 = ops.gemm_tma_vt(out[:B].view(B * S, C), w["wkv_c"].bf16, w["bkv_c"], C, S, slot=2)
        hid = ops.attn_tc(kq1, C, k0, 0, vt0, B, NUM_HEADS, S, S, d, scale, out_dtype=torch.bfloat16)
        _tail_bf16(x1, hid, w["tail_cross"], out=out[B:].view(B * S, C))
        return out

    @torch.no_grad()
    def forward(self, feats0, embeddings0, feats1, embeddings1, masks0=None, masks1=None):
        if masks0 is not None or masks1 is not None:
            raise NotImplementedError("key masks are never used on the SAM-6D inference path")
        w = self._weights()
        emb = _stack2(embeddings0, embeddings1) if feats0.shape == feats1.shape else None
        if emb is not None and self.precision == "bf16" and feats0.shape[1] <= 256:
            B = feats0.shape[0]
            f = _stack2(feats0, feats1)
            if f is None:
                f = torch.cat([feats0, feats1], dim=0)
            f = self._forward_bf16(f.to(torch.bfloat16).contiguous(), emb, w)
            return f[:B], f[B:]
        if emb is not None:
            B = feats0.shape[0]
            f = _stack2(feats0, feats1)
            f = self._self_layer(f if f is not None else torch.cat([feats0, feats1], dim=0), emb, w)
            feats0, feats1 = f[:B], f[B:]
        else:
            feats0 = self._self_layer(feats0.contiguous(), embeddings0, w)
            feats1 = self._self_layer(feats1.contiguous(), embeddings1, w)
        feats0 = self._cross_layer(feats0, feats1, w)
        feats1 = self._cross_layer(feats1, feats0, w)
        return feats0, feats1


class _SinusoidalBuffer(nn.Module):
    def __init__(self, d_model):
        super().__init__()
        div_indices = torch.arange(0, d_model, 2).float()
        self.register_buffer('div_term', torch.exp(div_indices * (-math.log(10000.0) / d_model)))


class GeometricStructureEmbedding(nn.Module):

    def __init__(self, cfg):
        super().__init__()
        cfg = _cfg(cfg)
        self.sigma_d, self.sigma_a, self.angle_k = cfg.sigma_d, cfg.sigma_a, cfg.angle_k
        self.factor_a = 180.0 / (self.sigma_a * math.pi)
        if cfg.reduction_a != 'max' or cfg.angle_k != 3 or cfg.hidden_dim != 256:
            raise ValueError("sam6d_b200 kernels are built for reduction_a='max', angle_k=3, hidden_dim=256")
        self.embedding = _SinusoidalBuffer(cfg.hidden_dim)
        self.proj_d = nn.Linear(cfg.hidden_dim, cfg.hidden_dim)
        self.proj_a = nn.Linear(cfg.hidden_dim, cfg.hidden_dim)
        self._packed = _Packed()
        self.precision = "fp32"

    def _weights(self):
        key = _param_key(self)
        if self._packed.key != key:
            self._packed.w = dict(div=_f32(self.embedding.div_term), waT=_f32(self.proj_a.weight).t().contiguous(),
                                  wdT=_f32(self.proj_d.weight).t().contiguous(),
                                  wd_bf=_f32(self.proj_d.weight).to(torch.bfloat16).contiguous(),
                                  bias=(_f32(self.proj_a.bias) + _f32(self.proj_d.bias)).contiguous())
            self._packed.w.update(self._tables(self._packed.w))
            self._packed.key = key
        return self._packed.w

    def _tables(self, w):
        div = w["div"].double()

        def table(weight, x_max, bias=None):
            n = int(math.ceil(x_max * GEO_LUT_INV_H)) + 1
            om = (torch.arange(n, dtype=torch.float64, device=div.device) / GEO_LUT_INV_H)[:, None] * div[None, :]
            emb = torch.stack([torch.sin(om), torch.cos(om)], dim=2).reshape(n, -1)
            g = emb @ weight.detach().double().t()
            if bias is not None:
                g = g + bias.double()
            return g.to(torch.float32).to(torch.bfloat16).contiguous()

        return dict(tab_a=table(self.proj_a.weight, 180.0 / self.sigma_a), tab_d=table(self.proj_d.weight, GEO_LUT_D_MAX, w["bias"]),
                    wdT_bf=_f32(self.proj_d.weight).t().contiguous().to(torch.bfloat16).contiguous())

    @torch.no_grad()
    def get_embedding_indices(self, points):
        T = ops.geo_indices(points.contiguous(), self.sigma_d, self.factor_a)
        return T[..., 3], T[..., :3]

    @torch.no_grad()
    def forward(self, points):
        w = self._weights()
        T = ops.geo_indices(points.contiguous(), self.sigma_d, self.factor_a)
        if self.precision == "bf16":
            far = ops.geo_embed_dist_tc(torch.stack([T[:, 0, :, :], T[:, :, 0, :]], dim=1).contiguous(), w["div"], w["wd_bf"], w["bias"])
            return ops.geo_embed_lut(T, w["tab_a"], GEO_LUT_INV_H, w["tab_d"], GEO_LUT_INV_H, far, w["div"], w["wdT_bf"], w["bias"])
        return ops.geo_embed_f32(T, w["div"], w["waT"], w["wdT"], w["bias"])


def sample_pts_feats(pts, feats, npoint=2048, return_index=False):
    idx = ops.furthest_point_sampling(pts.contiguous(), npoint)
    p = ops.gather_rows(pts.contiguous(), idx)
    f = ops.gather_rows_bf16_f32(feats.contiguous(), idx) if feats.dtype == torch.bfloat16 else ops.gather_rows(feats.contiguous(), idx)
    return (p, f, idx) if return_index else (p, f)


def compute_feature_similarity(feat1, feat2, type='cosine', temp=1.0, normalize_feat=True, precision="fp32"):
    if type != 'cosine':
        raise NotImplementedError("SAM-6D uses sim_type='cosine'")
    B, N, C = feat1.shape
    M = feat2.shape[1]
    ld = (M + 3) // 4 * 4
    store = torch.empty(B, N, ld, dtype=torch.float32, device=feat1.device)
    if precision == "bf16":
        f1 = ops.l2norm_rows_bf16(feat1.contiguous()) if normalize_feat else feat1.contiguous().to(torch.bfloat16)
        f2 = ops.l2norm_rows_bf16(feat2.contiguous()) if normalize_feat else feat2.contiguous().to(torch.bfloat16)
        ops.gemm_tma_batched(f1, f2, store, N, M, ld, N * ld, alpha=1.0 / temp)
    else:
        f1 = ops.l2norm_rows(feat1.contiguous()) if normalize_feat else feat1.contiguous()
        f2 = ops.l2norm_rows(feat2.contiguous()) if normalize_feat else feat2.contiguous()
        ops.gemm_raw(f1.data_ptr(), f2.data_ptr(), None, 0, store.data_ptr(), N, M, C, C, C, ld, 0, batch=B, sA=N * C, sW=M * C,
                     sC=N * ld, alpha=1.0 / temp)
    return store[:, :, :M]


def compute_coarse_Rt(atten, pts1, pts2, model_pts=None, n_proposal1=6000, n_proposal2=300, rand=None, return_scores=False):
    B = pts1.shape[0]
    if model_pts is None:
        model_pts = pts2
    W, w1 = ops.coarse_assign(atten.contiguous())
    if rand is None:
        rand = torch.rand(B, n_proposal1 * 3, device=pts1.device)
    idx = ops.coarse_sample(W, rand.contiguous())
    Rt, resid = ops.coarse_hypotheses(idx, pts1.contiguous(), pts2.contiguous())
    top = ops.topk_smallest(resid, n_proposal2)
    R, t, scores = ops.coarse_select(Rt, top, pts1.contiguous(), w1, model_pts.contiguous())
    if return_scores:
        return R, t, scores
    return R, t


def compute_fine_Rt(atten, pts1, pts2, model_pts=None, dis_thres=0.15, temp=0.1, radius=None, check_bound=True):
    if model_pts is None:
        model_pts = pts2
    bound = 1.0 / temp
    if check_bound and float(atten.abs().max()) > bound * (1.0 + 1e-3):
        raise ValueError(f"compute_fine_Rt: |atten| exceeds 1/temp = {bound:g}; the CUDA path handles cosine scores "
                         "(sim_type='cosine', normalize_feat=True) only")
    pts1, pts2 = pts1.contiguous(), pts2.contiguous()
    lab1, _, wts, pred = ops.fine_assign(atten, pts2, shift=1.0 / temp)
    R, t = ops.weighted_procrustes(pred, pts1, wts, 0.0, 1e-5)
    rad = radius if radius is not None else torch.ones(pts1.shape[0], device=pts1.device) - 1e-6
    score, t_scaled = ops.pose_score(pts1, lab1, R, t, model_pts.contiguous(), rad.contiguous(), dis_thres)
    return (R, t, score) if radius is None else (R, t, score, t_scaled)


class CoarsePointMatching(nn.Module):

    def __init__(self, cfg, return_feat=False):
        super().__init__()
        self.cfg = _cfg(cfg)
        self.return_feat = return_feat
        self.nblock = self.cfg.nblock
        self.in_proj = nn.Linear(self.cfg.input_dim, self.cfg.hidden_dim)
        self.out_proj = nn.Linear(self.cfg.hidden_dim, self.cfg.out_dim)
        self.bg_token = nn.Parameter(torch.randn(1, 1, self.cfg.hidden_dim) * .02)
        self.transformers = nn.ModuleList([
            GeometricTransformer(blocks=['self', 'cross'], d_model=self.cfg.hidden_dim, num_heads=4, dropout=None,
                                 activation_fn='ReLU', return_attention_scores=False) for _ in range(self.nblock)])
        self._packed = _Packed()
        self.precision = "fp32"

    def _weights(self):
        key = _param_key(self.in_proj) + _param_key(self.out_proj)
        if self._packed.key != key:
            self._packed.w = dict(w_in=_W(self.in_proj.weight), b_in=_f32(self.in_proj.bias), w_out=_W(self.out_proj.weight),
                                  b_out=_f32(self.out_proj.bias))
            self._packed.key = key
        return self._packed.w

    def _embed(self, f):
        B, n, C = f.shape
        w = self._weights()
        H = self.cfg.hidden_dim
        if self.precision == "bf16":
            out = torch.empty(B, n + 1, H, dtype=torch.bfloat16, device=f.device)
            out[:, 0, :] = self.bg_token.detach().reshape(1, -1).to(torch.bfloat16)
            ops.gemm_tc_raw(f.data_ptr(), 0, w["w_in"].bf16.data_ptr(), 1, w["b_in"], 0, out.data_ptr() + H * 2, 1, n, H, C, C, C, H, 0,
                            batch=B, sA=n * C, sW=0, sC=(n + 1) * H)
            return out
        out = torch.empty(B, n + 1, H, dtype=torch.float32, device=f.device)
        out[:, 0, :] = self.bg_token.detach().reshape(1, -1)
        _gemm_raw(self.precision, f.data_ptr(), w["w_in"], w["b_in"], 0, out.data_ptr() + H * 4, n, H, C, C, H, 0, batch=B,
                  sA=n * C, sC=(n + 1) * H)
        return out

    @torch.no_grad()
    def forward(self, p1, f1, geo1, p2, f2, geo2, radius, end_points, rand=None):
        if self.training:
            raise NotImplementedError("sam6d_b200 implements the inference path (model.eval())")
        f12 = _stack2(f1, f2)
        if f12 is not None:
            e = self._embed(f12)
            f1, f2 = e[:f1.shape[0]], e[f1.shape[0]:]
        else:
            f1 = self._embed(f1.contiguous())
            f2 = self._embed(f2.contiguous())
        for blk in self.transformers:
            f1, f2 = blk(f1, geo1, f2, geo2)
        B, S, H = f1.shape
        w = self._weights()
        f12 = _stack2(f1, f2)
        if f12 is not None:
            o = _gemm(self.precision, f12.reshape(2 * B * S, H), w["w_out"], w["b_out"]).view(2 * B, S, -1)
            o1, o2 = o[:B], o[B:]
        else:
            o1 = _gemm(self.precision, f1.reshape(B * S, H), w["w_out"], w["b_out"]).view(B, S, -1)
            o2 = _gemm(self.precision, f2.reshape(B * S, H), w["w_out"], w["b_out"]).view(B, S, -1)
        atten = compute_feature_similarity(o1, o2, self.cfg.sim_type, self.cfg.temp, self.cfg.normalize_feat, self.precision)
        model = ops.scale_by_radius(end_points['model'].contiguous(), radius.contiguous())
        init_R, init_t, self.last_select_scores = compute_coarse_Rt(atten, p1, p2, model, self.cfg.nproposal1,
                                                                    self.cfg.nproposal2, rand=rand, return_scores=True)
        end_points['init_R'] = init_R
        end_points['init_t'] = init_t
        if self.return_feat:
            return end_points, o1, o2
        return end_points


class _ConvBN(nn.Module):

    def __init__(self, cin, cout):
        super().__init__()
        self.conv = nn.Conv2d(cin, cout, kernel_size=(1, 1), bias=False)
        self.normlayer = nn.Module()
        self.normlayer.bn = nn.BatchNorm2d(cout)

    def folded(self):
        bn = self.normlayer.bn
        w = self.conv.weight.detach().double().reshape(self.conv.out_channels, -1)
        s = bn.weight.detach().double() / torch.sqrt(bn.running_var.detach().double() + bn.eps)
        return (w * s[:, None]).float().contiguous(), (bn.bias.detach().double() - bn.running_mean.detach().double() * s).float().contiguous()


class _SharedMLP(nn.Module):
    def __init__(self, dims):
        super().__init__()
        for i in range(len(dims) - 1):
            self.add_module(f"layer{i}", _ConvBN(dims[i], dims[i + 1]))


class _Conv1dParams(nn.Module):
    def __init__(self, cin, cout):
        super().__init__()
        self.conv = nn.Conv1d(cin, cout, kernel_size=1, bias=True)


class PositionalEncoding(nn.Module):

    def __init__(self, out_dim, r1=0.1, r2=0.2, nsample1=32, nsample2=64, use_xyz=True, bn=True):
        super().__init__()
        if not (use_xyz and bn) or (nsample1, nsample2) != (32, 64):
            raise ValueError("sam6d_b200 PositionalEncoding is built for the SAM-6D configuration")
        self.r1, self.r2, self.ns1, self.ns2 = r1, r2, nsample1, nsample2
        self.mlp1 = _SharedMLP([6, 32, 64, 128])
        self.mlp2 = _SharedMLP([6, 32, 64, 128])
        self.mlp3 = _Conv1dParams(256, out_dim)
        self._packed = _Packed()
        self.precision = "fp32"

    def _weights(self):
        key = _param_key(self)
        if self._packed.key != key:
            w = {}
            for name, mlp in (("m1", self.mlp1), ("m2", self.mlp2)):
                packed = []
                for j in range(3):
                    wj, bj = getattr(mlp, f"layer{j}").folded()
                    packed += [wj, bj]
                w[name] = tuple(packed)
                w[name + "_tc"] = (packed[0], packed[1], packed[2].to(torch.bfloat16).contiguous(), packed[3],
                                   packed[4].to(torch.bfloat16).contiguous(), packed[5])
            w["w3"] = _W(_f32(self.mlp3.conv.weight).reshape(self.mlp3.conv.out_channels, -1))
            w["b3"] = _f32(self.mlp3.conv.bias)
            self._packed.w, self._packed.key = w, key
        return self._packed.w

    @torch.no_grad()
    def local_features(self, pts):
        w = self._weights()
        pts = pts.contiguous()
        B, N, _ = pts.shape
        feat = torch.empty(B, N, 256, dtype=torch.bfloat16 if self.precision == "bf16" else torch.float32, device=pts.device)
        pair = ops.ball_query_pair(pts, pts, self.r1, self.ns1, self.r2, self.ns2) if self.r1 <= self.r2 else None
        for r, ns, name, off in ((self.r1, self.ns1, "m1", 0), (self.r2, self.ns2, "m2", 128)):
            if pair is not None:
                idx, cnt = pair[:2] if off == 0 else pair[2:]
            else:
                idx, cnt = ops.ball_query(pts, pts, r, ns, return_count=True)
            if self.precision == "bf16":
                ops.pe_mlp_max_tc(pts, idx, w[name + "_tc"], feat, off)
            else:
                ops.pe_mlp_max(pts, idx, cnt, w[name], feat, off)
        return feat

    @torch.no_grad()
    def forward(self, pts1, pts2=None):
        if pts2 is not None and pts2 is not pts1:
            raise NotImplementedError("SAM-6D always calls PE(pts) with a single cloud")
        w = self._weights()
        feat = self.local_features(pts1)
        B, N, _ = feat.shape
        if self.precision == "bf16":
            return ops.gemm_tma(feat.view(B * N, 256), w["w3"].bf16, w["b3"]).view(B, N, -1)
        return _gemm(self.precision, feat.view(B * N, 256), w["w3"], w["b3"]).view(B, N, -1)


class _LinearAttentionParams(nn.Module):
    def __init__(self, d_model):
        super().__init__()
        self.proj_q = nn.Linear(d_model, d_model)
        self.proj_k = nn.Linear(d_model, d_model)
        self.proj_v = nn.Linear(d_model, d_model)
        self.scale = nn.Parameter(torch.zeros(size=(1, 1, d_model)))


class _LinearAttentionLayerParams(nn.Module):
    def __init__(self, d_model):
        super().__init__()
        self.attention = _LinearAttentionParams(d_model)
        self.linear = nn.Linear(d_model, d_model)
        self.norm = nn.LayerNorm(d_model)


class _LinearTransformerLayerParams(nn.Module):
    def __init__(self, d_model):
        super().__init__()
        self.attention = _LinearAttentionLayerParams(d_model)
        self.output = _AttentionOutputParams(d_model)


class SparseToDenseTransformer(nn.Module):

    def __init__(self, d_model, sparse_blocks, num_heads=4, dropout=None, activation_fn='ReLU', parallel=False,
                 focusing_factor=3, with_bg_token=True, replace_bg_token=True):
        super().__init__()
        if not (with_bg_token and replace_bg_token) or focusing_factor != 3:
            raise ValueError("sam6d_b200 SparseToDenseTransformer is built for the SAM-6D configuration")
        self.d_model = d_model
        self.sparse_layer = GeometricTransformer(blocks=sparse_blocks, d_model=d_model, num_heads=num_heads, dropout=dropout,
                                                 activation_fn=activation_fn, parallel=parallel, return_attention_scores=False)
        self.dense_layer = _LinearTransformerLayerParams(d_model)
        self._packed = _Packed()
        self.precision = "fp32"

    def _weights(self):
        key = _param_key(self.dense_layer)
        if self._packed.key != key:
            la = self.dense_layer.attention.attention
            self._packed.w = dict(
                wq=_W(la.proj_q.weight), bq=_f32(la.proj_q.bias),
                wkv=_W(torch.cat([_f32(la.proj_k.weight), _f32(la.proj_v.weight)], dim=0)),
                bkv=torch.cat([_f32(la.proj_k.bias), _f32(la.proj_v.bias)], dim=0).contiguous(),
                sp_scale=torch.nn.functional.softplus(_f32(la.scale)).reshape(-1).contiguous(), tail=_pack_tail(self.dense_layer))
            self._packed.key = key
        return self._packed.w

    def _sample_feats(self, dense_feats, idx_ext):
        if dense_feats.dtype == torch.bfloat16:
            return ops.gather_rows_bf16(dense_feats, idx_ext)
        return ops.gather_rows(dense_feats, idx_ext)

    def _dense_layer_bf16(self, dense, sparse, w):
        B, N1, C = dense.shape
        N, J = N1 - 1, sparse.shape[1] - 1
        dev = dense.device
        bf = torch.bfloat16
        x2d = dense.view(B * N1, C)
        q = ops.gemm_tma(x2d, w["wq"].bf16, w["bq"], out_dtype=bf)
        kv = torch.empty(B * J, 2 * C, dtype=torch.float32, device=dev)
        s_bf = sparse.dtype == torch.bfloat16
        ops.gemm_tc_raw(sparse.data_ptr() + C * (2 if s_bf else 4), int(s_bf), w["wkv"].bf16.data_ptr(), 1, w["bkv"], 0, kv.data_ptr(), 0,
                        J, 2 * C, C, C, C, 2 * C, 0, batch=B, sA=(J + 1) * C, sW=0, sC=J * 2 * C)
        ops.focus_rows_raw(kv.data_ptr(), (B * J, 0, 2 * C), kv.data_ptr(), (B * J, 0, 2 * C), w["sp_scale"], B * J, C)
        blob, KS = ops.linattn_kv_pack_raw(kv.data_ptr(), 2 * C, J * 2 * C, kv.data_ptr() + C * 4, 2 * C, J * 2 * C, B, J, dev)
        x_att = torch.empty(B * N1, C, dtype=bf, device=dev)
        ops.linattn_tc_raw(q.data_ptr() + C * 2, C, N1 * C, blob, KS, w["sp_scale"], B, N, x_att.data_ptr() + C * 2, C, N1 * C)
        x_att.view(B, N1, C)[:, 0, :] = 0
        out = _tail_bf16(x2d, x_att, w["tail"]).view(B, N1, C)
        out[:, 0, :] = sparse[:, 0, :].to(bf)
        return out

    def _dense_layer(self, dense, sparse, w):
        B, N1, C = dense.shape
        N, J = N1 - 1, sparse.shape[1] - 1
        f = 4
        dev = dense.device
        x_ptr, x_view = dense.data_ptr() + C * f, (N, N1 * C, C)
        q = torch.empty(B * N, C, dtype=torch.float32, device=dev)
        prec = self.precision
        _gemm_raw(prec, x_ptr, w["wq"], w["bq"], 0, q.data_ptr(), N, C, C, C, C, 0, batch=B, sA=N1 * C, sC=N * C)
        kv = torch.empty(B * J, 2 * C, dtype=torch.float32, device=dev)
        _gemm_raw(prec, sparse.data_ptr() + C * f, w["wkv"], w["bkv"], 0, kv.data_ptr(), J, 2 * C, C, C, 2 * C, 0, batch=B,
                  sA=(J + 1) * C, sC=J * 2 * C)
        ops.focus_rows_raw(q.data_ptr(), (B * N, 0, C), q.data_ptr(), (B * N, 0, C), w["sp_scale"], B * N, C)
        ops.focus_rows_raw(kv.data_ptr(), (B * J, 0, 2 * C), kv.data_ptr(), (B * J, 0, 2 * C), w["sp_scale"], B * J, C)
        KV = torch.empty(B, NUM_HEADS, 64, 64, dtype=torch.float32, device=dev)
        KS = torch.empty(B, NUM_HEADS, 64, dtype=torch.float32, device=dev)
        ops.linattn_kv_raw(kv.data_ptr(), 2 * C, J * 2 * C, kv.data_ptr() + C * f, 2 * C, J * 2 * C, B, NUM_HEADS, J, KV, KS)
        x_att = torch.empty(B * N, C, dtype=torch.float32, device=dev)
        ops.linattn_apply_raw(q.data_ptr(), N, N * C, C, KV, KS, B, NUM_HEADS, x_att.data_ptr(), N * C, C)
        t = w["tail"]
        y = torch.empty(B * N, C, dtype=torch.float32, device=dev)
        _gemm_raw(prec, x_att.data_ptr(), t["wo"], t["bo"], x_ptr, y.data_ptr(), N, C, C, C, C, C, batch=B, sA=N * C, sC=N * C,
                  sR=N1 * C)
        y = ops.layernorm(y, t["g1"], t["b1"])
        h = _gemm(prec, y, t["we"], t["be"], relu=True)
        z = _gemm(prec, h, t["ws"], t["bs"], residual=y)
        out = torch.empty(B, N1, C, dtype=torch.float32, device=dev)
        ops.layernorm_raw(z.data_ptr(), (B * N, 0, C), out.data_ptr() + C * f, (N, N1 * C, C), t["g2"], t["b2"], B * N, C)
        out[:, 0, :] = sparse[:, 0, :]
        return out

    @torch.no_grad()
    def forward(self, dense_feats0, embeddings0, fps_idx0, dense_feats1, embeddings1, fps_idx1, masks0=None, masks1=None):
        w = self._weights()
        ext0 = torch.cat([torch.zeros_like(fps_idx0[:, :1]), fps_idx0], dim=1).contiguous()
        ext1 = torch.cat([torch.zeros_like(fps_idx1[:, :1]), fps_idx1], dim=1).contiguous()
        dense = _stack2(dense_feats0, dense_feats1)
        if dense is not None:
            B = dense_feats0.shape[0]
            feats = self._sample_feats(dense, torch.cat([ext0, ext1], dim=0))
            feats0, feats1 = self.sparse_layer(feats[:B], embeddings0, feats[B:], embeddings1, masks0, masks1)
            layer = self._dense_layer_bf16 if dense.dtype == torch.bfloat16 else self._dense_layer
            out = layer(dense, torch.cat([feats0, feats1], dim=0), w)
            return out[:B], out[B:]
        feats0 = self._sample_feats(dense_feats0.contiguous(), ext0)
        feats1 = self._sample_feats(dense_feats1.contiguous(), ext1)
        feats0, feats1 = self.sparse_layer(feats0, embeddings0, feats1, embeddings1, masks0, masks1)
        layer = self._dense_layer_bf16 if dense_feats0.dtype == torch.bfloat16 else self._dense_layer
        dense_feats0 = layer(dense_feats0.contiguous(), feats0, w)
        dense_feats1 = layer(dense_feats1.contiguous(), feats1, w)
        return dense_feats0, dense_feats1


class FinePointMatching(nn.Module):

    def __init__(self, cfg, return_feat=False):
        super().__init__()
        self.cfg = _cfg(cfg)
        self.return_feat = return_feat
        self.nblock = self.cfg.nblock
        self.in_proj = nn.Linear(self.cfg.input_dim, self.cfg.hidden_dim)
        self.out_proj = nn.Linear(self.cfg.hidden_dim, self.cfg.out_dim)
        self.bg_token = nn.Parameter(torch.randn(1, 1, self.cfg.hidden_dim) * .02)
        self.PE = PositionalEncoding(self.cfg.hidden_dim, r1=self.cfg.pe_radius1, r2=self.cfg.pe_radius2)
        self._packed = _Packed()
        self.precision = "fp32"
        self.transformers = nn.ModuleList([
            SparseToDenseTransformer(self.cfg.hidden_dim, num_heads=4, sparse_blocks=['self', 'cross'], dropout=None,
                                     activation_fn='ReLU', focusing_factor=self.cfg.focusing_factor, with_bg_token=True,
                                     replace_bg_token=True) for _ in range(self.nblock)])

    def _weights(self):
        key = _param_key(self.in_proj) + _param_key(self.out_proj)
        if self._packed.key != key:
            self._packed.w = dict(w_in=_W(self.in_proj.weight), b_in=_f32(self.in_proj.bias), w_out=_W(self.out_proj.weight),
                                  b_out=_f32(self.out_proj.bias))
            self._packed.key = key
        return self._packed.w

    def _embed(self, f, pts):
        B, N, C = f.shape
        H = self.cfg.hidden_dim
        w, pw = self._weights(), self.PE._weights()
        local = self.PE.local_features(pts)
        if self.precision == "bf16":
            f2d = f.reshape(B * N, C)
            if f2d.dtype == torch.bfloat16 and f2d.is_contiguous():
                tmp = ops.gemm_tma(f2d, w["w_in"].bf16, w["b_in"], out_dtype=torch.bfloat16)
            else:
                tmp = ops.gemm_tc(f2d, w["w_in"].bf16, w["b_in"], out_dtype=torch.bfloat16)
            out = torch.empty(B, N + 1, H, dtype=torch.bfloat16, device=f.device)
            out[:, 0, :] = self.bg_token.detach().reshape(1, -1).to(torch.bfloat16)
            ops.gemm_tma_batched(local, pw["w3"].bf16, out[:, 1:, :], N, H, H, (N + 1) * H, bias=pw["b3"],
                                 residual=tmp.view(B, N, H), ldr=H, r_bs=N * H)
            return out
        tmp = _gemm(self.precision, f.reshape(B * N, C), w["w_in"], w["b_in"])
        out = torch.empty(B, N + 1, H, dtype=torch.float32, device=f.device)
        out[:, 0, :] = self.bg_token.detach().reshape(1, -1)
        _gemm_raw(self.precision, local.data_ptr(), pw["w3"], pw["b3"], tmp.data_ptr(), out.data_ptr() + H * 4, N, H, 256, 256, H, H,
                  batch=B, sA=N * 256, sC=(N + 1) * H, sR=N * H)
        return out

    @torch.no_grad()
    def forward(self, p1, f1, geo1, fps_idx1, p2, f2, geo2, fps_idx2, radius, end_points):
        if self.training:
            raise NotImplementedError("sam6d_b200 implements the inference path (model.eval())")
        p1, p2 = p1.contiguous(), p2.contiguous()
        p1_ = ops.rigid_warp(p1, end_points['init_R'].contiguous(), end_points['init_t'].contiguous())
        f12 = _stack2(f1, f2) if p1.shape == p2.shape else None
        if f12 is not None:
            e = self._embed(f12, torch.cat([p1_, p2], dim=0))
            f1, f2 = e[:p1.shape[0]], e[p1.shape[0]:]
        else:
            f1 = self._embed(f1.contiguous(), p1_)
            f2 = self._embed(f2.contiguous(), p2)
        for blk in self.transformers:
            f1, f2 = blk(f1, geo1, fps_idx1, f2, geo2, fps_idx2)
        B, S, H = f1.shape
        w = self._weights()
        f12 = _stack2(f1, f2)
        if f12 is not None:
            o = _gemm(self.precision, f12.reshape(2 * B * S, H), w["w_out"], w["b_out"]).view(2 * B, S, -1)
            o1, o2 = o[:B], o[B:]
        else:
            o1 = _gemm(self.precision, f1.reshape(B * S, H), w["w_out"], w["b_out"]).view(B, S, -1)
            o2 = _gemm(self.precision, f2.reshape(B * S, H), w["w_out"], w["b_out"]).view(B, S, -1)
        model = ops.scale_by_radius(end_points['model'].contiguous(), radius.contiguous())
        if (self.precision == "bf16" and self.cfg.sim_type == 'cosine' and self.cfg.normalize_feat and H == 256
                and o1.shape[-1] == 256 and not self.return_feat):
            f1n, f2n = ops.l2norm_rows_bf16(o1.contiguous()), ops.l2norm_rows_bf16(o2.contiguous())
            lab1, _, wts, pred = ops.fine_assign_tc(f1n, f2n, p2, 1.0 / self.cfg.temp)
            pred_R, pred_t = ops.weighted_procrustes(pred, p1, wts, 0.0, 1e-5)
            score, t_scaled = ops.pose_score(p1, lab1, pred_R, pred_t, model.contiguous(), radius.contiguous(), 0.15)
        else:
            if not self.cfg.normalize_feat:
                raise NotImplementedError("FinePointMatching: normalize_feat=False scores are unbounded; the fixed-shift assignment "
                                          "kernels need cosine similarities (the SAM-6D configuration)")
            atten = compute_feature_similarity(o1, o2, self.cfg.sim_type, self.cfg.temp, self.cfg.normalize_feat, self.precision)
            pred_R, _, score, t_scaled = compute_fine_Rt(atten, p1, p2, model, temp=self.cfg.temp, radius=radius.contiguous(),
                                                         check_bound=False)
        end_points['pred_R'] = pred_R
        end_points['pred_t'] = t_scaled
        end_points['pred_pose_score'] = score
        if self.return_feat:
            return end_points, o1, o2
        return end_points


DEFAULT_MODEL_CFG = dict(
    coarse_npoint=196, fine_npoint=2048,
    geo_embedding=dict(sigma_d=0.2, sigma_a=15, angle_k=3, reduction_a='max', hidden_dim=256),
    coarse_point_matching=dict(nblock=3, input_dim=256, hidden_dim=256, out_dim=256, temp=0.1, sim_type='cosine',
                               normalize_feat=True, loss_dis_thres=0.15, nproposal1=6000, nproposal2=300),
    fine_point_matching=dict(nblock=3, input_dim=256, hidden_dim=256, out_dim=256, pe_radius1=0.1, pe_radius2=0.2,
                             focusing_factor=3, temp=0.1, sim_type='cosine', normalize_feat=True, loss_dis_thres=0.15),
)


class Net(nn.Module):

    def __init__(self, cfg=None, feature_extraction: Optional[nn.Module] = None, precision: str = "fp32"):
        super().__init__()
        cfg = _cfg(cfg if cfg is not None else DEFAULT_MODEL_CFG)
        self.cfg = cfg
        self.coarse_npoint = cfg.coarse_npoint
        self.fine_npoint = cfg.fine_npoint
        if feature_extraction is not None:
            self.feature_extraction = feature_extraction
        elif hasattr(cfg, "feature_extraction"):
            from .vit import ViTEncoder
            self.feature_extraction = ViTEncoder(cfg.feature_extraction, cfg.fine_npoint, precision)
        self.geo_embedding = GeometricStructureEmbedding(cfg.geo_embedding)
        self.coarse_point_matching = CoarsePointMatching(cfg.coarse_point_matching)
        self.fine_point_matching = FinePointMatching(cfg.fine_point_matching)
        self._graphs = None
        self.set_precision(precision)

    def enable_graphs(self, max_graphs: int = 8):
        from .graph import StepGraphs
        self._graphs = StepGraphs(max_graphs)
        return self

    def disable_graphs(self):
        self._graphs = None
        return self

    def set_precision(self, precision: str):
        if precision not in PRECISIONS:
            raise ValueError(f"precision must be one of {PRECISIONS}")
        self.precision = precision
        for m in self.modules():
            if hasattr(m, "precision") and m is not self:
                m.precision = precision
        return self

    def _features(self, end_points):
        if 'dense_fm' in end_points:
            dense_fm = end_points['dense_fm']
        elif hasattr(self, 'feature_extraction'):
            dense_fm = self.feature_extraction.get_img_feats(end_points['rgb'], end_points['rgb_choose'])
        else:
            raise RuntimeError("Net needs end_points['dense_fm'] or a feature_extraction module for the RGB branch")
        if 'dense_po' not in end_points or 'dense_fo' not in end_points:
            raise RuntimeError("inference needs the template bank: end_points['dense_po'], end_points['dense_fo']")
        dense_po = end_points['dense_po'].contiguous()
        radius = ops.cloud_radius(dense_po)
        dense_pm = ops.scale_by_radius(end_points['pts'].contiguous(), radius)
        dense_po = ops.scale_by_radius(dense_po, radius)
        return dense_pm, dense_fm.contiguous(), dense_po, end_points['dense_fo'].contiguous(), radius

    @torch.no_grad()
    def forward(self, end_points, rand=None, init_pose=None):
        if self.training:
            raise NotImplementedError("sam6d_b200 implements the inference path: call model.eval()")
        if self._graphs is not None and init_pose is None and 'pts' in end_points:
            n_rand = self.coarse_point_matching.cfg.nproposal1 * 3
            out = self._graphs.run(lambda ep, r: self._forward(ep, r, None), end_points, rand, n_rand,
                                   extra=(self.precision, hash(_param_key(self))))
            if out is not None:
                return out
        return self._forward(end_points, rand, init_pose)

    def _forward(self, end_points, rand, init_pose):
        dense_pm, dense_fm, dense_po, dense_fo, radius = self._features(end_points)
        B = dense_pm.size(0)
        if dense_pm.shape == dense_po.shape and dense_fm.shape == dense_fo.shape:
            pts2 = torch.cat([dense_pm, dense_po], dim=0)
            if self.precision == "bf16":
                fts2 = torch.empty(2 * B, *dense_fm.shape[1:], dtype=torch.bfloat16, device=dense_fm.device)
                fts2[:B].copy_(dense_fm)
                fts2[B:].copy_(dense_fo)
            else:
                fts2 = torch.cat([dense_fm, dense_fo], dim=0)
            dense_pm, dense_po, dense_fm, dense_fo = pts2[:B], pts2[B:], fts2[:B], fts2[B:]
            sp, sf, idx = sample_pts_feats(pts2, fts2, self.coarse_npoint, return_index=True)
            bg_point = torch.ones(2 * B, 1, 3, dtype=torch.float32, device=pts2.device) * 100
            geo = self.geo_embedding(torch.cat([bg_point, sp], dim=1))
            sparse_pm, sparse_po, sparse_fm, sparse_fo = sp[:B], sp[B:], sf[:B], sf[B:]
            fps_idx_m, fps_idx_o, geo_embedding_m, geo_embedding_o = idx[:B], idx[B:], geo[:B], geo[B:]
        else:
            bg_point = torch.ones(B, 1, 3, dtype=torch.float32, device=dense_pm.device) * 100
            sparse_pm, sparse_fm, fps_idx_m = sample_pts_feats(dense_pm, dense_fm, self.coarse_npoint, return_index=True)
            geo_embedding_m = self.geo_embedding(torch.cat([bg_point, sparse_pm], dim=1))
            sparse_po, sparse_fo, fps_idx_o = sample_pts_feats(dense_po, dense_fo, self.coarse_npoint, return_index=True)
            geo_embedding_o = self.geo_embedding(torch.cat([bg_point, sparse_po], dim=1))
        end_points = self.coarse_point_matching(sparse_pm, sparse_fm, geo_embedding_m, sparse_po, sparse_fo, geo_embedding_o,
                                                radius, end_points, rand=rand)
        if init_pose is not None:
            coarse_R, coarse_t = end_points['init_R'], end_points['init_t']
            end_points['init_R'], end_points['init_t'] = init_pose[0].contiguous(), init_pose[1].contiguous()
        end_points = self.fine_point_matching(dense_pm, dense_fm, geo_embedding_m, fps_idx_m, dense_po, dense_fo,
                                              geo_embedding_o, fps_idx_o, radius, end_points)
        if init_pose is not None:
            end_points['init_R'], end_points['init_t'] = coarse_R, coarse_t
        return end_points
```

Baseline: 2624.

## Skip empty ball-query neighbor groups in PE MLP and split fine-pass edge row/column

The bf16 point-embedding MLP now uses ball-query counts to pack only occupied 8-neighbor groups into a compacted descriptor list, so the tensor-core kernel no longer runs padded duplicate neighbors. This adds two small pack/compact kernels and a per-call workspace allocation. Separately, the fine matching passes treat row/column 0 (the background token) outside the tiled GEMM. They take precomputed edge dot products and a dedicated row-0 reduction kernel, shrinking the main tile range by one. This adds extra launches and a new edge-dot kernel.

```diff
diff --git a/include/sam6d_b200.h b/include/sam6d_b200.h
--- a/include/sam6d_b200.h
+++ b/include/sam6d_b200.h
@@ -172,10 +172,15 @@
 int sam6d_pe_mlp_max_tc(const float* pts, const int* idx, int B, int N, int ns, const float* W1, const float* B1,
                         const void* W2_bf16, const float* B2, const void* W3_bf16, const float* B3, void* out, int out_is_bf16,
                         int out_ld, int out_off, void* stream);
+int sam6d_pe_mlp_max_tc_cnt(const float* pts, const int* idx, const int* cnt, int B, int N, int ns, const float* W1,
+                            const float* B1, const void* W2_bf16, const float* B2, const void* W3_bf16, const float* B3, void* out,
+                            int out_is_bf16, int out_ld, int out_off, int* work, long long work_len, void* stream);
 int sam6d_fine_assign(const float* A, int B, int S, int ld, float shift, const float* pts2, float* rsum, float* csum, float* cpart,
                       int* cpi, int* lab1, int* lab2, float* wts, float* pred, void* stream);
 int sam6d_fine_pass_tc(const void* Fa, const void* Fb, int B, int S, float alpha, float shift, int mode, const float* row_f,
-                       const float* col_f, int ld_f, const float* q4, float* out_inv, int* lab, float* wts, float* pred, void* stream);
+                       const float* col_f, int ld_f, const float* q4, const float* c0, const float* r0, float* out_inv, int* lab,
+                       float* wts, float* pred, void* stream);
+int sam6d_fine_edge_dots(const void* F1, const void* F2, int B, int S, int ld, float* dcol, float* drow, void* stream);
 int sam6d_fine_masked_points(const int* lab2, const float* pts2, int B, int S, int ld, float* q4, void* stream);
 int sam6d_weighted_procrustes(const float* src, const float* ref, const float* wts, int B, int N, float weight_thresh,
                               float eps, float* R, float* t, void* stream);
diff --git a/sam6d_b200/_lib.py b/sam6d_b200/_lib.py
--- a/sam6d_b200/_lib.py
+++ b/sam6d_b200/_lib.py
@@ -58,7 +58,7 @@
 
 
 _launches = 0
-_MULTI = {"sam6d_fine_assign": 6, "sam6d_coarse_select": 2, "sam6d_geo_embed_tc": 2, "sam6d_render_meshes": 4, "sam6d_yolo_masks": 2,
+_MULTI = {"sam6d_fine_assign": 6, "sam6d_fine_pass_tc": 2, "sam6d_pe_mlp_max_tc_cnt": 3, "sam6d_coarse_select": 2, "sam6d_geo_embed_tc": 2, "sam6d_render_meshes": 4, "sam6d_yolo_masks": 2,
           "sam6d_mask_rle_count": 2}
 _timed = {}
 
diff --git a/sam6d_b200/csrc/fine_tc.cu b/sam6d_b200/csrc/fine_tc.cu
--- a/sam6d_b200/csrc/fine_tc.cu
+++ b/sam6d_b200/csrc/fine_tc.cu
@@ -17,6 +17,7 @@
   const float* row_f;
   const float* col_f;
   const float4* q4;
+  const float* c0;
   float* out_inv;
   int* lab;
   float* wts; float* pred;
@@ -39,7 +40,7 @@
   __shared__ __align__(16) float4 sq[2][BN];
 
   const int tid = threadIdx.x, warp = tid >> 5, lane = tid & 31;
-  const int m_tiles = (g.S + BM - 1) / BM, n_tiles = (g.S + BN - 1) / BN;
+  const int m_tiles = (g.S - 1 + BM - 1) / BM, n_tiles = (g.S - 1 + BN - 1) / BN;
   const int items = g.B * m_tiles;
 
   if (tid == 0) {
@@ -60,13 +61,13 @@
         const int b = item / m_tiles, mt = item - b * m_tiles;
         tc::mbar_wait(&a_empty, (uint32_t)((it & 1) ^ 1));
         tc::mbar_arrive_expect_tx(&a_full, KB * A_KB);
-        for (int kb = 0; kb < KB; ++kb) tc::tma_load_2d(&tmA, &a_full, a_res + kb * A_KB, kb * BK, b * g.S + mt * BM);
+        for (int kb = 0; kb < KB; ++kb) tc::tma_load_2d(&tmA, &a_full, a_res + kb * A_KB, kb * BK, b * g.S + 1 + mt * BM);
         for (int nt = 0; nt < n_tiles; ++nt)
           for (int kb = 0; kb < KB; ++kb, ++gk) {
             const int s = (int)(gk % STAGES);
             tc::mbar_wait(&empty_bar[s], (uint32_t)(((gk / STAGES) & 1) ^ 1));
             tc::mbar_arrive_expect_tx(&full_bar[s], B_KB);
-            tc::tma_load_2d(&tmB, &full_bar[s], ring + s * B_KB, kb * BK, b * g.S + nt * BN);
+            tc::tma_load_2d(&tmB, &full_bar[s], ring + s * B_KB, kb * BK, b * g.S + 1 + nt * BN);
           }
       }
     }
@@ -82,18 +83,30 @@
     float rf[2] = {0.f, 0.f};
 #pragma unroll
     for (int hr = 0; hr < 2; ++hr) {
-      const int i = mt * BM + wg * 64 + tc::frag_row(2 * hr, w, lane);
+      const int i = 1 + mt * BM + wg * 64 + tc::frag_row(2 * hr, w, lane);
       if (MODE != 0 && i < g.S) rf[hr] = g.row_f[(size_t)b * g.ld_f + i];
     }
     const float* cf = (MODE != 0) ? g.col_f + (size_t)b * g.ld_f : nullptr;
     const float4* q4 = (MODE == 2) ? g.q4 + (size_t)b * g.ld_f : nullptr;
     float sum[2] = {0.f, 0.f}, bv[2] = {-INFINITY, -INFINITY}, ws[2] = {0.f, 0.f}, px[2] = {0.f, 0.f}, py[2] = {0.f, 0.f}, pz[2] = {0.f, 0.f};
     int bi[2] = {0x7fffffff, 0x7fffffff};
+#pragma unroll
+    for (int hr = 0; hr < 2; ++hr) {
+      const int i = 1 + mt * BM + wg * 64 + tc::frag_row(2 * hr, w, lane);
+      if (i >= g.S) continue;
+      const float ev = ex2(fmaf(g.c0[(size_t)b * g.ld_f + i], g.a2, -g.s2));
+      if (MODE == 0) {
+        if ((lane & 3) == 0) sum[hr] = ev;
+      } else {
+        bv[hr] = (ev * rf[hr]) * (ev * cf[0]);
+        bi[hr] = 0;
+      }
+    }
     tc::mbar_wait(&a_full, (uint32_t)(it & 1));
     for (int nt = 0; nt < n_tiles; ++nt, ++tcount) {
       const int buf = (int)(tcount & 1);
       if (MODE != 0) {
-        const int j = nt * BN + tid;
+        const int j = 1 + nt * BN + tid;
         sc[buf][tid] = (j < g.S) ? cf[j] : 0.f;
         if (MODE == 2) sq[buf][tid] = (j < g.S) ? q4[j] : make_float4(0.f, 0.f, 0.f, 0.f);
         tc::named_bar(1, CONSUMERS);
@@ -120,7 +133,7 @@
       if (nt == n_tiles - 1 && lane == 0) tc::mbar_arrive(&a_empty);
 #pragma unroll
       for (int e = 0; e < BN / 2; ++e) {
-        const int hr = (e >> 1) & 1, cl = tc::frag_col(e, lane), j = nt * BN + cl;
+        const int hr = (e >> 1) & 1, cl = tc::frag_col(e, lane), j = 1 + nt * BN + cl;
         const float ev = (j < g.S) ? ex2(fmaf(acc[e], g.a2, -g.s2)) : 0.f;
         if (MODE == 0) {
           sum[hr] += ev;
@@ -137,7 +150,7 @@
     }
 #pragma unroll
     for (int hr = 0; hr < 2; ++hr) {
-      const int i = mt * BM + wg * 64 + tc::frag_row(2 * hr, w, lane);
+      const int i = 1 + mt * BM + wg * 64 + tc::frag_row(2 * hr, w, lane);
       if (MODE == 0) {
         const float t = tc::quad_sum(sum[hr]);
         if ((lane & 3) == 0 && i < g.S) g.out_inv[(size_t)b * g.ld_f + i] = 1.f / t;
@@ -167,6 +180,76 @@
   }
 }
 
+__global__ void __launch_bounds__(256) fine_edge_dots_kernel(const __nv_bfloat16* __restrict__ F1, const __nv_bfloat16* __restrict__ F2,
+                                                             int S, int ld, float* __restrict__ dcol, float* __restrict__ drow) {
+  const int b = blockIdx.y, lane = threadIdx.x & 31, i = blockIdx.x * 8 + (threadIdx.x >> 5);
+  if (i >= S) return;
+  auto dot8 = [&](const __nv_bfloat16* x, const __nv_bfloat16* y) {
+    const uint4 u = *reinterpret_cast<const uint4*>(x + lane * 8), v = *reinterpret_cast<const uint4*>(y + lane * 8);
+    const __nv_bfloat162* xu = reinterpret_cast<const __nv_bfloat162*>(&u);
+    const __nv_bfloat162* yv = reinterpret_cast<const __nv_bfloat162*>(&v);
+    float acc = 0.f;
+#pragma unroll
+    for (int k = 0; k < 4; ++k) {
+      const float2 xf = __bfloat1622float2(xu[k]), yf = __bfloat1622float2(yv[k]);
+      acc = fmaf(xf.x, yf.x, acc);
+      acc = fmaf(xf.y, yf.y, acc);
+    }
+    return acc;
+  };
+  const __nv_bfloat16* f1 = F1 + (size_t)b * S * 256;
+  const __nv_bfloat16* f2 = F2 + (size_t)b * S * 256;
+  float c = dot8(f1 + (size_t)i * 256, f2), r = dot8(f1, f2 + (size_t)i * 256);
+#pragma unroll
+  for (int o = 16; o > 0; o >>= 1) {
+    c += __shfl_xor_sync(0xffffffffu, c, o);
+    r += __shfl_xor_sync(0xffffffffu, r, o);
+  }
+  if (lane == 0) { dcol[(size_t)b * ld + i] = c; drow[(size_t)b * ld + i] = r; }
+}
+
+template <int MODE>
+__global__ void __launch_bounds__(256) fine_row0_kernel(const float* __restrict__ r0, FArgs g) {
+  __shared__ float sv[8];
+  __shared__ int si[8];
+  const int b = blockIdx.x, tid = threadIdx.x, lane = tid & 31, warp = tid >> 5;
+  const float* r = r0 + (size_t)b * g.ld_f;
+  const float rf = (MODE != 0) ? g.row_f[(size_t)b * g.ld_f] : 0.f;
+  float sum = 0.f, bv = -INFINITY;
+  int bi = 0x7fffffff;
+  for (int j = tid; j < g.S; j += blockDim.x) {
+    const float ev = ex2(fmaf(r[j], g.a2, -g.s2));
+    if (MODE == 0) {
+      sum += ev;
+    } else {
+      const float p = (ev * rf) * (ev * g.col_f[(size_t)b * g.ld_f + j]);
+      if (p > bv) { bv = p; bi = j; }
+    }
+  }
+#pragma unroll
+  for (int o = 16; o > 0; o >>= 1) {
+    if (MODE == 0) {
+      sum += __shfl_xor_sync(0xffffffffu, sum, o);
+    } else {
+      const float ov = __shfl_xor_sync(0xffffffffu, bv, o);
+      const int oi = __shfl_xor_sync(0xffffffffu, bi, o);
+      if (ov > bv || (ov == bv && oi < bi)) { bv = ov; bi = oi; }
+    }
+  }
+  if (lane == 0) { sv[warp] = MODE == 0 ? sum : bv; si[warp] = bi; }
+  __syncthreads();
+  if (tid == 0) {
+    float t = sv[0];
+    int ti = si[0];
+    for (int w = 1; w < 8; ++w) {
+      if (MODE == 0) t += sv[w];
+      else if (sv[w] > t || (sv[w] == t && si[w] < ti)) { t = sv[w]; ti = si[w]; }
+    }
+    if (MODE == 0) g.out_inv[(size_t)b * g.ld_f] = 1.f / t;
+    else g.lab[(size_t)b * g.S] = ti == 0x7fffffff ? 0 : ti;
+  }
+}
+
 typedef CUresult (*EncodeFn)(CUtensorMap*, CUtensorMapDataType, cuuint32_t, void*, const cuuint64_t*, const cuuint64_t*,
                              const cuuint32_t*, const cuuint32_t*, CUtensorMapInterleave, CUtensorMapSwizzle,
                              CUtensorMapL2promotion, CUtensorMapFloatOOBfill);
@@ -208,9 +291,9 @@
 }
 
 S6_API int sam6d_fine_pass_tc(const void* Fa, const void* Fb, int B, int S, float alpha, float shift, int mode, const float* row_f,
-                              const float* col_f, int ld_f, const float* q4, float* out_inv, int* lab, float* wts, float* pred,
-                              void* stream) {
-  S6_REQUIRE(Fa && Fb && B >= 0 && S >= 2 && mode >= 0 && mode <= 2 && ld_f >= S);
+                              const float* col_f, int ld_f, const float* q4, const float* c0, const float* r0, float* out_inv, int* lab,
+                              float* wts, float* pred, void* stream) {
+  S6_REQUIRE(Fa && Fb && c0 && r0 && B >= 0 && S >= 2 && mode >= 0 && mode <= 2 && ld_f >= S);
   S6_REQUIRE(((reinterpret_cast<uintptr_t>(Fa) | reinterpret_cast<uintptr_t>(Fb)) & 15) == 0 && (long long)B * S < 2000000000LL);
   if (mode == 0) S6_REQUIRE(out_inv != nullptr);
   if (mode >= 1) S6_REQUIRE(row_f && col_f && lab);
@@ -224,13 +307,14 @@
   int dev = 0, sms = 0;
   S6_CHECK(cudaGetDevice(&dev));
   S6_CHECK(cudaDeviceGetAttribute(&sms, cudaDevAttrMultiProcessorCount, dev));
-  const int items = B * s6_cdiv(S, BM);
+  const int items = B * s6_cdiv(S - 1, BM);
   const int grid = items < sms ? items : sms;
-  FArgs g{B, S, mode, ld_f, alpha * LOG2E, shift * LOG2E, row_f, col_f, reinterpret_cast<const float4*>(q4), out_inv, lab, wts, pred};
+  FArgs g{B, S, mode, ld_f, alpha * LOG2E, shift * LOG2E, row_f, col_f, reinterpret_cast<const float4*>(q4), c0, out_inv, lab, wts, pred};
   cudaStream_t st = s6_stream(stream);
 #define FINE_LAUNCH(M)                                                                                              \
   do {                                                                                                              \
     S6_CHECK(cudaFuncSetAttribute(fine_pass_kernel<M>, cudaFuncAttributeMaxDynamicSharedMemorySize, SMEM_BYTES));   \
+    fine_row0_kernel<M><<<B, 256, 0, st>>>(r0, g);                                                                  \
     fine_pass_kernel<M><<<grid, NUM_THREADS, SMEM_BYTES, st>>>(tmA, tmB, g);                                        \
   } while (0)
   if (mode == 0) FINE_LAUNCH(0); else if (mode == 1) FINE_LAUNCH(1); else FINE_LAUNCH(2);
@@ -247,3 +331,14 @@
   S6_LAUNCH_CHECK();
   return 0;
 }
+
+S6_API int sam6d_fine_edge_dots(const void* F1, const void* F2, int B, int S, int ld, float* dcol, float* drow, void* stream) {
+  S6_REQUIRE(F1 && F2 && dcol && drow && B >= 0 && S >= 2 && ld >= S);
+  S6_REQUIRE(((reinterpret_cast<uintptr_t>(F1) | reinterpret_cast<uintptr_t>(F2)) & 15) == 0);
+  if (B == 0) return 0;
+  dim3 grid(s6_cdiv(S, 8), B);
+  fine_edge_dots_kernel<<<grid, 256, 0, s6_stream(stream)>>>(reinterpret_cast<const __nv_bfloat16*>(F1),
+                                                            reinterpret_cast<const __nv_bfloat16*>(F2), S, ld, dcol, drow);
+  S6_LAUNCH_CHECK();
+  return 0;
+}
diff --git a/sam6d_b200/csrc/pe_tc.cu b/sam6d_b200/csrc/pe_tc.cu
--- a/sam6d_b200/csrc/pe_tc.cu
+++ b/sam6d_b200/csrc/pe_tc.cu
@@ -14,9 +14,20 @@
 __device__ __forceinline__ void st_feat(float* p, float v) { *p = v; }
 __device__ __forceinline__ void st_feat(__nv_bfloat16* p, float v) { *p = __float2bfloat16(v); }
 
+constexpr int GROUPS = ROWS / 8;
+
+template <int NS>
+__device__ __forceinline__ int fixed_desc(long long t, int g, long long total_points) {
+  constexpr int GPP = NS / 8;
+  const long long gp = t * (ROWS / NS) + g / GPP;
+  const int k = g % GPP;
+  return gp < total_points ? (int)((gp << 4) | ((k == GPP - 1) << 3) | k) : -1;
+}
+
 template <int NS, typename OT>
 __global__ void __launch_bounds__(NUM_THREADS, 4) pe_tc_kernel(const float* __restrict__ pts, const int* __restrict__ idx, int N,
-                                                               long long total_points,
+                                                               long long total_points, const int* __restrict__ desc,
+                                                               const int* __restrict__ ntiles_dev,
                                                                const float* __restrict__ W1, const float* __restrict__ B1,
                                                                const __nv_bfloat16* __restrict__ W2, const float* __restrict__ B2,
                                                                const __nv_bfloat16* __restrict__ W3, const float* __restrict__ B3,
@@ -26,12 +37,13 @@
   uint8_t* a1 = smem;
   uint8_t* a2 = a1 + SLAB;
   uint8_t* w3s = a2 + SLAB;
+  float* gmax = reinterpret_cast<float*>(a1 + 64 * 128);
   __shared__ __align__(16) float w1s[32 * 8];
   __shared__ __align__(16) float b1s[32], b2s[64], b3s[128];
+  __shared__ int sdesc[2][GROUPS];
 
   const int tid = threadIdx.x, warp = tid >> 5, lane = tid & 31;
-  constexpr int PPT = ROWS / NS;
-  const long long ntiles = (total_points + PPT - 1) / PPT;
+  const long long ntiles = desc ? (long long)*ntiles_dev : (total_points + ROWS / NS - 1) / (ROWS / NS);
 
   for (int e = tid; e < 32 * 8; e += NUM_THREADS) { int r = e >> 3, c = e & 7; w1s[e] = (c < 6) ? W1[r * 6 + c] : 0.f; }
   if (tid < 32) b1s[tid] = B1[tid];
@@ -51,14 +63,16 @@
   {
     const int r = tid;
     const uint32_t a1_addr = tc::smem_u32(a1), a2_addr = tc::smem_u32(a2), w2_addr = tc::smem_u32(a1) + 64, w3_addr = tc::smem_u32(w3s);
-    auto load_idx = [&](long long tile) -> int {
-      const long long gp = tile * PPT + r / NS;
-      return (tile < ntiles && gp < total_points) ? __ldg(idx + gp * NS + (r % NS)) : -1;
+    auto load_desc = [&](long long tile) -> int {
+      if (tile >= ntiles) return -1;
+      return desc ? __ldg(desc + tile * GROUPS + (r >> 3)) : fixed_desc<NS>(tile, r >> 3, total_points);
     };
-    auto load_x = [&](long long tile, int j, float (&xx)[6]) {
-      const long long gp = tile * PPT + r / NS;
+    auto load_idx = [&](int d) -> int {
+      return d >= 0 ? __ldg(idx + (long long)(d >> 4) * NS + ((d & 7) << 3) + (r & 7)) : -1;
+    };
+    auto load_x = [&](int d, int j, float (&xx)[6]) {
       if (j >= 0) {
-        const long long b = gp / N;
+        const long long gp = d >> 4, b = gp / N;
         const float* pi = pts + gp * 3;
         const float* pj = pts + (b * N + j) * 3;
         const float jx = __ldg(pj), jy = __ldg(pj + 1), jz = __ldg(pj + 2);
@@ -69,10 +83,16 @@
       }
     };
     float xn[6];
-    load_x(blockIdx.x, load_idx(blockIdx.x), xn);
-    int jn = load_idx((long long)blockIdx.x + gridDim.x);
-    for (long long tile = blockIdx.x; tile < ntiles; tile += gridDim.x) {
+    int dx = load_desc(blockIdx.x);
+    load_x(dx, load_idx(dx), xn);
+    int d1 = load_desc((long long)blockIdx.x + gridDim.x);
+    int jn = load_idx(d1);
+    int d2 = load_desc((long long)blockIdx.x + 2LL * gridDim.x);
+    int it = 0;
+    for (long long tile = blockIdx.x; tile < ntiles; tile += gridDim.x, ++it) {
+      int* sd = sdesc[it & 1];
       {
+        if ((r & 7) == 0) sd[r >> 3] = dx;
         float x[6];
 #pragma unroll
         for (int e = 0; e < 6; ++e) x[e] = xn[e];
@@ -118,8 +138,11 @@
       }
       tc::fence_proxy_async_smem();
       worker_bar();
-      load_x(tile + gridDim.x, jn, xn);
-      jn = load_idx(tile + 2LL * gridDim.x);
+      load_x(d1, jn, xn);
+      dx = d1;
+      jn = load_idx(d2);
+      d1 = d2;
+      d2 = load_desc(tile + 3LL * gridDim.x);
 #pragma unroll
       for (int blk = 0; blk < 2; ++blk) {
         float acc[64];
@@ -131,38 +154,109 @@
         tc::wg_wait<0>();
 #pragma unroll
         for (int hr = 0; hr < 2; ++hr) {
-          const int ch = blk * 64 + tc::frag_row(2 * hr, warp, lane);
-          const float bias = b3s[ch];
-#pragma unroll
-          for (int p = 0; p < PPT; ++p) {
-            constexpr int JG = NS / 8;
-            float m = -INFINITY;
-#pragma unroll
-            for (int j = p * JG; j < (p + 1) * JG; ++j) m = fmaxf(m, fmaxf(acc[4 * j + 2 * hr], acc[4 * j + 2 * hr + 1]));
-            m = tc::quad_max(m);
-            const long long p_out = tile * PPT + p;
-            if ((lane & 3) == 0 && p_out < total_points) st_feat(out + p_out * out_ld + out_off + ch, fmaxf(m + bias, 0.f));
+          const int ch = blk * 64 + tc::frag_row(2 * hr, warp, lane), b0 = lane & 1, b1 = (lane >> 1) & 1;
+          float w8[8], u4[4];
+#pragma unroll
+          for (int k = 0; k < 8; ++k) {
+            const float ve = fmaxf(acc[8 * k + 2 * hr], acc[8 * k + 2 * hr + 1]);
+            const float vo = fmaxf(acc[8 * k + 4 + 2 * hr], acc[8 * k + 4 + 2 * hr + 1]);
+            w8[k] = fmaxf(b0 ? vo : ve, __shfl_xor_sync(0xffffffffu, b0 ? ve : vo, 1));
+          }
+#pragma unroll
+          for (int k = 0; k < 4; ++k) u4[k] = fmaxf(b1 ? w8[2 * k + 1] : w8[2 * k], __shfl_xor_sync(0xffffffffu, b1 ? w8[2 * k] : w8[2 * k + 1], 2));
+#pragma unroll
+          for (int k = 0; k < 4; ++k) gmax[(4 * k + 2 * b1 + b0) * 128 + (ch ^ ((2 * b1 + b0) << 3))] = u4[k];
+        }
+      }
+      worker_bar();
+      {
+        const int ch = tid;
+        const float bias = b3s[ch];
+        float m = -INFINITY;
+#pragma unroll
+        for (int g = 0; g < GROUPS; ++g) {
+          m = fmaxf(m, gmax[g * 128 + (ch ^ ((g & 3) << 3))]);
+          const int d = sd[g];
+          if (d >= 0 && (d & 8)) {
+            st_feat(out + (long long)(d >> 4) * out_ld + out_off + ch, fmaxf(m + bias, 0.f));
+            m = -INFINITY;
           }
         }
       }
+      worker_bar();
     }
   }
 }
 
-}
-
-S6_API int sam6d_pe_mlp_max_tc(const float* pts, const int* idx, int B, int N, int ns, const float* W1, const float* B1,
-                               const void* W2_bf16, const float* B2, const void* W3_bf16, const float* B3, void* out, int out_is_bf16,
-                               int out_ld, int out_off, void* stream) {
-  S6_REQUIRE(pts && idx && W1 && B1 && W2_bf16 && B2 && W3_bf16 && B3 && out && B >= 0 && N > 0);
-  S6_REQUIRE(ns == 32 || ns == 64);
-  if (B == 0) return 0;
+constexpr int SEG = 256;
+template <int NS>
+__global__ void __launch_bounds__(128) pe_pack_kernel(const int* __restrict__ cnt, int N, int nseg, int* __restrict__ loc,
+                                                      int* __restrict__ ntile) {
+  const int lane = threadIdx.x & 31, sgi = blockIdx.x * 4 + (threadIdx.x >> 5);
+  if (sgi >= nseg) return;
+  const int spc = (N + SEG - 1) / SEG, b = sgi / spc, p0 = (sgi - b * spc) * SEG, pn = min(SEG, N - p0);
+  int* tl = loc + (size_t)sgi * (2 * NS) * GROUPS;
+  int gv[SEG / 32];
+#pragma unroll
+  for (int c = 0; c < SEG / 32; ++c) {
+    const int k = c * 32 + lane;
+    gv[c] = k < pn ? (min(max(__ldg(cnt + (size_t)b * N + p0 + k), 1), NS) + 7) >> 3 : 0;
+  }
+  int tile = 0, fill = 0;
+#pragma unroll
+  for (int c = 0; c < SEG / 32; ++c) {
+    const int k = c * 32 + lane, g = gv[c];
+    int incl = g;
+#pragma unroll
+    for (int o = 1; o < 32; o <<= 1) {
+      const int v = __shfl_up_sync(0xffffffffu, incl, o);
+      if (lane >= o) incl += v;
+    }
+    const int excl = incl - g;
+    int s = 0, run0 = 0, my_tile = 0, my_off = 0;
+    while (true) {
+      const unsigned over = __ballot_sync(0xffffffffu, lane >= s && fill + incl - run0 > GROUPS);
+      const int e = over ? __ffs(over) - 1 : 32;
+      if (lane >= s && lane < e) { my_tile = tile; my_off = fill + excl - run0; }
+      if (!over) { fill += __shfl_sync(0xffffffffu, incl, 31) - run0; break; }
+      const int ex = __shfl_sync(0xffffffffu, excl, e);
+      const int used = fill + ex - run0;
+      if (lane >= used && lane < GROUPS) tl[(size_t)tile * GROUPS + lane] = -1;
+      ++tile; fill = 0; s = e; run0 = ex;
+    }
+    const long long gp = (long long)b * N + p0 + k;
+    for (int q = 0; q < g; ++q) tl[(size_t)my_tile * GROUPS + my_off + q] = (int)((gp << 4) | ((q == g - 1) << 3) | q);
+  }
+  if (fill > 0 && lane >= fill && lane < GROUPS) tl[(size_t)tile * GROUPS + lane] = -1;
+  if (lane == 0) ntile[sgi] = tile + (fill > 0);
+}
+
+__global__ void __launch_bounds__(128) pe_compact_kernel(const int* __restrict__ loc, const int* __restrict__ ntile, int nseg, int tseg,
+                                                         int* __restrict__ desc, int* __restrict__ ntiles_out) {
+  __shared__ int part[4];
+  const int b = blockIdx.x, tid = threadIdx.x;
+  int s = 0;
+  for (int i = tid; i < b; i += blockDim.x) s += ntile[i];
+#pragma unroll
+  for (int o = 16; o > 0; o >>= 1) s += __shfl_xor_sync(0xffffffffu, s, o);
+  if ((tid & 31) == 0) part[tid >> 5] = s;
+  __syncthreads();
+  const long long base = part[0] + part[1] + part[2] + part[3];
+  const int n = ntile[b];
+  const int4* src = reinterpret_cast<const int4*>(loc + (size_t)b * tseg * GROUPS);
+  int4* dst = reinterpret_cast<int4*>(desc + base * GROUPS);
+  for (int i = tid; i < n * (GROUPS / 4); i += blockDim.x) dst[i] = src[i];
+  if (b == nseg - 1 && tid == 0) *ntiles_out = (int)(base + n);
+}
+
+int pe_launch(const float* pts, const int* idx, const int* desc, const int* ntiles_dev, int B, int N, int ns, const float* W1,
+              const float* B1, const void* W2_bf16, const float* B2, const void* W3_bf16, const float* B3, void* out, int out_is_bf16,
+              int out_ld, int out_off, cudaStream_t st) {
   int dev = 0, sms = 0;
   S6_CHECK(cudaGetDevice(&dev));
   S6_CHECK(cudaDeviceGetAttribute(&sms, cudaDevAttrMultiProcessorCount, dev));
   const long long total = (long long)B * N;
   const long long ntiles = (total + (128 / ns) - 1) / (128 / ns);
-  cudaStream_t st = s6_stream(stream);
   const __nv_bfloat16* W2 = reinterpret_cast<const __nv_bfloat16*>(W2_bf16);
   const __nv_bfloat16* W3 = reinterpret_cast<const __nv_bfloat16*>(W3_bf16);
 #define PE_LAUNCH(NSV, OT)                                                                                                          \
@@ -174,7 +268,7 @@
        \
     const int per_sm = 4;                                                                                                           \
     const int grid = (int)(ntiles < (long long)sms * per_sm ? ntiles : (long long)sms * per_sm);                                    \
-    pe_tc_kernel<NSV, OT><<<grid, NUM_THREADS, SMEM_BYTES, st>>>(pts, idx, N, total, W1, B1, W2, B2, W3, B3,                         \
+    pe_tc_kernel<NSV, OT><<<grid, NUM_THREADS, SMEM_BYTES, st>>>(pts, idx, N, total, desc, ntiles_dev, W1, B1, W2, B2, W3, B3,       \
                                                                  reinterpret_cast<OT*>(out), out_ld, out_off);                      \
   } while (0)
   if (ns == 32) { if (out_is_bf16) PE_LAUNCH(32, __nv_bfloat16); else PE_LAUNCH(32, float); }
@@ -183,3 +277,39 @@
   S6_LAUNCH_CHECK();
   return 0;
 }
+
+}
+
+S6_API int sam6d_pe_mlp_max_tc(const float* pts, const int* idx, int B, int N, int ns, const float* W1, const float* B1,
+                               const void* W2_bf16, const float* B2, const void* W3_bf16, const float* B3, void* out, int out_is_bf16,
+                               int out_ld, int out_off, void* stream) {
+  S6_REQUIRE(pts && idx && W1 && B1 && W2_bf16 && B2 && W3_bf16 && B3 && out && B >= 0 && N > 0);
+  S6_REQUIRE(ns == 32 || ns == 64);
+  S6_REQUIRE((long long)B * N < (1LL << 27));
+  if (B == 0) return 0;
+  return pe_launch(pts, idx, nullptr, nullptr, B, N, ns, W1, B1, W2_bf16, B2, W3_bf16, B3, out, out_is_bf16, out_ld, out_off,
+                   s6_stream(stream));
+}
+
+S6_API int sam6d_pe_mlp_max_tc_cnt(const float* pts, const int* idx, const int* cnt, int B, int N, int ns, const float* W1,
+                                   const float* B1, const void* W2_bf16, const float* B2, const void* W3_bf16, const float* B3,
+                                   void* out, int out_is_bf16, int out_ld, int out_off, int* work, long long work_len, void* stream) {
+  S6_REQUIRE(pts && idx && cnt && W1 && B1 && W2_bf16 && B2 && W3_bf16 && B3 && out && work && B >= 0 && N > 0);
+  S6_REQUIRE(ns == 32 || ns == 64);
+  S6_REQUIRE((long long)B * N < (1LL << 27) && (reinterpret_cast<uintptr_t>(work) & 15) == 0);
+  const int nseg = B * s6_cdiv(N, SEG);
+  const long long slab = (long long)nseg * (2 * ns) * GROUPS;
+  S6_REQUIRE(work_len >= 2 * slab + nseg + 1);
+  if (B == 0) return 0;
+  int* desc = work;
+  int* loc = work + slab;
+  int* ntile = loc + slab;
+  int* ntiles = ntile + nseg;
+  cudaStream_t st = s6_stream(stream);
+  if (ns == 32) pe_pack_kernel<32><<<s6_cdiv(nseg, 4), 128, 0, st>>>(cnt, N, nseg, loc, ntile);
+  else pe_pack_kernel<64><<<s6_cdiv(nseg, 4), 128, 0, st>>>(cnt, N, nseg, loc, ntile);
+  S6_LAUNCH_CHECK();
+  pe_compact_kernel<<<nseg, 128, 0, st>>>(loc, ntile, nseg, 2 * ns, desc, ntiles);
+  S6_LAUNCH_CHECK();
+  return pe_launch(pts, idx, desc, ntiles, B, N, ns, W1, B1, W2_bf16, B2, W3_bf16, B3, out, out_is_bf16, out_ld, out_off, st);
+}
diff --git a/sam6d_b200/ops.py b/sam6d_b200/ops.py
--- a/sam6d_b200/ops.py
+++ b/sam6d_b200/ops.py
@@ -646,7 +646,7 @@
               _p(out), out.shape[-1], int(out_off), _s())
 
 
-def pe_mlp_max_tc(pts: Tensor, idx: Tensor, weights, out: Tensor, out_off: int):
+def pe_mlp_max_tc(pts: Tensor, idx: Tensor, weights, out: Tensor, out_off: int, cnt: Optional[Tensor] = None):
     _check(pts, torch.float32, "pts", 3)
     _check(idx, torch.int32, "idx", 3)
     B, N, _ = pts.shape
@@ -656,8 +656,15 @@
     _check(W3, torch.bfloat16, "W3", 2)
     if out.dtype not in (torch.float32, torch.bfloat16):
         raise RuntimeError("pe_mlp_max_tc: out must be float32 or bfloat16")
-    _lib.call("sam6d_pe_mlp_max_tc", _p(pts), _p(idx), B, N, ns, _p(W1), _p(B1), _p(W2), _p(B2), _p(W3), _p(B3), _p(out),
-              int(out.dtype == torch.bfloat16), out.shape[-1], int(out_off), _s())
+    tail = (_p(out), int(out.dtype == torch.bfloat16), out.shape[-1], int(out_off))
+    if cnt is None:
+        _lib.call("sam6d_pe_mlp_max_tc", _p(pts), _p(idx), B, N, ns, _p(W1), _p(B1), _p(W2), _p(B2), _p(W3), _p(B3), *tail, _s())
+        return
+    _check(cnt, torch.int32, "cnt", 2)
+    nseg = B * -(-N // 256)
+    work = torch.empty(2 * nseg * 2 * ns * 16 + nseg + 1, dtype=torch.int32, device=pts.device)
+    _lib.call("sam6d_pe_mlp_max_tc_cnt", _p(pts), _p(idx), _p(cnt), B, N, ns, _p(W1), _p(B1), _p(W2), _p(B2), _p(W3), _p(B3), *tail,
+              _p(work), work.numel(), _s())
 
 
 def fine_assign(A: Tensor, pts2: Tensor, shift: float):
@@ -704,13 +711,18 @@
     lab2 = torch.zeros(B, S, dtype=torch.int32, device=dev)
     wts = torch.empty(B, S - 1, dtype=torch.float32, device=dev)
     pred = torch.empty(B, S - 1, 3, dtype=torch.float32, device=dev)
+    dcol = torch.empty(B, ld, dtype=torch.float32, device=dev)
+    drow = torch.empty(B, ld, dtype=torch.float32, device=dev)
     a, sh = _f(alpha), _f(alpha)
-    _lib.call("sam6d_fine_pass_tc", _p(f1n), _p(f2n), B, S, a, sh, 0, None, None, ld, None, _p(rinv), None, None, None, _s())
-    _lib.call("sam6d_fine_pass_tc", _p(f2n), _p(f1n), B, S, a, sh, 0, None, None, ld, None, _p(cinv), None, None, None, _s())
-    _lib.call("sam6d_fine_pass_tc", _p(f2n), _p(f1n), B, S, a, sh, 1, _p(cinv), _p(rinv), ld, None, None, _p(lab2), None, None, _s())
+    _lib.call("sam6d_fine_edge_dots", _p(f1n), _p(f2n), B, S, ld, _p(dcol), _p(drow), _s())
+    e12, e21 = (_p(dcol), _p(drow)), (_p(drow), _p(dcol))
+    _lib.call("sam6d_fine_pass_tc", _p(f1n), _p(f2n), B, S, a, sh, 0, None, None, ld, None, *e12, _p(rinv), None, None, None, _s())
+    _lib.call("sam6d_fine_pass_tc", _p(f2n), _p(f1n), B, S, a, sh, 0, None, None, ld, None, *e21, _p(cinv), None, None, None, _s())
+    _lib.call("sam6d_fine_pass_tc", _p(f2n), _p(f1n), B, S, a, sh, 1, _p(cinv), _p(rinv), ld, None, *e21, None, _p(lab2), None, None,
+              _s())
     _lib.call("sam6d_fine_masked_points", _p(lab2), _p(pts2), B, S, ld, _p(q4), _s())
-    _lib.call("sam6d_fine_pass_tc", _p(f1n), _p(f2n), B, S, a, sh, 2, _p(rinv), _p(cinv), ld, _p(q4), None, _p(lab1), _p(wts), _p(pred),
-              _s())
+    _lib.call("sam6d_fine_pass_tc", _p(f1n), _p(f2n), B, S, a, sh, 2, _p(rinv), _p(cinv), ld, _p(q4), *e12, None, _p(lab1), _p(wts),
+              _p(pred), _s())
     return lab1, lab2, wts, pred
 
 
diff --git a/sam6d_b200/pem.py b/sam6d_b200/pem.py
--- a/sam6d_b200/pem.py
+++ b/sam6d_b200/pem.py
@@ -526,7 +526,7 @@
             else:
                 idx, cnt = ops.ball_query(pts, pts, r, ns, return_count=True)
             if self.precision == "bf16":
-                ops.pe_mlp_max_tc(pts, idx, w[name + "_tc"], feat, off)
+                ops.pe_mlp_max_tc(pts, idx, w[name + "_tc"], feat, off, cnt=cnt)
             else:
                 ops.pe_mlp_max(pts, idx, cnt, w[name], feat, off)
         return feat
```

New measurement: 2697 (median of 6 runs). 2.8% higher.
